# rafaelsoStanford/State_Policy_DiffusionModel

Measured on AMD Instinct MI355X. Metric: denoise-steps/sec (B=4096, horizon=32), higher is better.
Workload: dtype f32 (split-fp16 MFMA operands, fp32 accumulate)

## Files before the change

include/spdm.h:

```cpp
#ifndef SPDM_H
#define SPDM_H

#include <stddef.h>
#include <stdint.h>

#ifdef __cplusplus
extern "C" {
#endif

#define SPDM_NAME_MAX 64
#define SPDM_ABI_VERSION 2

typedef enum {
    SPDM_OK = 0,
    SPDM_ERR_INVALID = -1,
    SPDM_ERR_HIP = -2,
    SPDM_ERR_STATE = -3,
    SPDM_ERR_MISSING = -4,
    SPDM_ERR_NOMEM = -5
} spdm_status;

typedef enum { SPDM_DDPM = 0, SPDM_DDIM = 1 } spdm_scheduler_kind;

typedef struct spdm_handle spdm_handle;

typedef struct {
    int32_t horizon;
    int32_t state_dim;
    int32_t cond_dim;
    int32_t time_dim;
    int32_t attention;
    int32_t max_batch;
    int32_t device;
    int32_t num_train_timesteps;
    int32_t flags;
} spdm_config;

#define SPDM_FLAG_DEBUG_KEEP 1
#define SPDM_FLAG_EXACT_FP32 2
#define SPDM_FLAG_SIMPLE_UNET 4

#define SPDM_FLAG_TRAIN 8

#define SPDM_FLAG_TRAIN_ATTENTION 16

#define SPDM_FLAG_TRAIN_SIMPLE 32

typedef struct {
    char     name[SPDM_NAME_MAX];
    uint64_t offset;
    uint64_t numel;
    int32_t  ndim;
    int32_t  shape[4];
} spdm_tensor_index;

int  spdm_abi_version(void);
const char* spdm_last_error(void);

int  spdm_create(const spdm_config* cfg, spdm_handle** out);
void spdm_destroy(spdm_handle* h);

int  spdm_load_weights(spdm_handle* h, const float* h_blob, size_t n_floats,
                       const spdm_tensor_index* h_index, int32_t n_index);

int  spdm_update_weights(spdm_handle* h, const float* d_blob, size_t n_floats, void* stream);

int  spdm_debug_weight_digest(const spdm_handle* h, uint64_t* out);

int  spdm_set_time_table(spdm_handle* h, const float* h_table, int32_t T);

int  spdm_set_schedule(spdm_handle* h, int32_t kind, int32_t num_train_timesteps,
                       int32_t num_inference_steps, float beta_start, float beta_end);

int  spdm_set_schedule_tables(spdm_handle* h, int32_t kind, int32_t n_steps,
                              const int32_t* h_timesteps, const float* h_coef);

int  spdm_schedule_tables(int32_t kind, int32_t num_train_timesteps, int32_t num_inference_steps,
                          float beta_start, float beta_end,
                          int32_t* h_timesteps_out, float* h_coef_out );

int  spdm_unet_forward(spdm_handle* h, int32_t B, const float* d_x, const int32_t* h_t,
                       int32_t t_count, const float* d_cond, float* d_eps, void* stream);

int  spdm_sample(spdm_handle* h, int32_t B, const float* d_cond,
                 const float* d_inpaint, int32_t inp_h, int32_t inpaint_per_sample,
                 const float* d_xT, const float* d_noise, uint64_t seed, uint64_t sample_offset,
                 float* d_out, float* d_history, void* stream);

int  spdm_train_loss_grad(spdm_handle* h, int32_t B, const float* d_x_noisy, const int32_t* h_t, int32_t t_count,
                          const float* d_cond, const float* d_noise, float* d_loss, float* d_eps, float* d_grad,
                          float* d_grad_cond, void* stream);

int  spdm_train_set_time_scale(spdm_handle* h, const float* d_scale, int32_t B);

int  spdm_sample_begin(spdm_handle* h, int32_t B, const float* d_cond,
                       const float* d_inpaint, int32_t inp_h, int32_t inpaint_per_sample,
                       const float* d_xT, const float* d_noise, uint64_t seed,
                       uint64_t sample_offset, float* d_history, void* stream);
int  spdm_sample_run(spdm_handle* h, int32_t step_begin, int32_t step_end, void* stream);
int  spdm_sample_result(spdm_handle* h, float* d_out, void* stream);

int64_t spdm_graph_captures(const spdm_handle* h);

int  spdm_debug_tensor(spdm_handle* h, const char* name, float* d_out, size_t cap_floats,
                       int32_t shape_out[4]);

int32_t spdm_demoted_tensors(const spdm_handle* h);
int  spdm_nonfinite(spdm_handle* h, int32_t* flag_out, void* stream);

int  spdm_set_switch(spdm_handle* h, const char* name, int32_t on);

int32_t spdm_uses_split_precision(const spdm_handle* h);

size_t spdm_device_bytes(const spdm_handle* h);

int  spdm_profile_enable(spdm_handle* h, int32_t on);
int  spdm_profile_read(spdm_handle* h, int64_t* launches, double* total_ms, double* total_flops);

int  spdm_bench_gemm(int32_t device, int32_t B, int32_t H, int32_t W, int32_t Cin, int32_t Cout, int32_t taps,
                     int32_t pro, int32_t epi, int32_t split, int32_t iters, int32_t debug,
                     double* ms_out );

typedef struct spdm_encoder spdm_encoder;
int  spdm_encoder_create(int32_t device, const float* h_blob, size_t n_floats, const spdm_tensor_index* h_index,
                         int32_t n_index, spdm_encoder** out);
int  spdm_encoder_forward(spdm_encoder* e, int32_t n_images, const float* d_images, float* d_latent, void* stream);
void spdm_encoder_destroy(spdm_encoder* e);

int  spdm_encoder_train_forward(spdm_encoder* e, int32_t n_images, const float* d_images, float* d_latent, void* stream);
int  spdm_encoder_backward(spdm_encoder* e, int32_t n_images, const float* d_images, const float* d_grad_latent,
                           float* d_grad, void* stream);
int  spdm_encoder_update_weights(spdm_encoder* e, const float* d_blob, size_t n_floats, void* stream);

typedef struct spdm_decoder spdm_decoder;
int  spdm_decoder_create(int32_t device, const float* h_blob, size_t n_floats, const spdm_tensor_index* h_index,
                         int32_t n_index, spdm_decoder** out);
int  spdm_decoder_forward(spdm_decoder* d, int32_t n, const float* d_latent, float* d_recon, void* stream);
int  spdm_decoder_train_loss(spdm_decoder* d, int32_t n, const float* d_latent, const float* d_target,
                             float* d_recon , float* d_loss, void* stream);
int  spdm_decoder_backward(spdm_decoder* d, int32_t n, const float* d_latent, const float* d_target, float* d_grad,
                           float* d_grad_latent, void* stream);
int  spdm_decoder_update_weights(spdm_decoder* d, const float* d_blob, size_t n_floats, void* stream);
void spdm_decoder_destroy(spdm_decoder* d);

#define SPDM_OPTIM_MAX_SEGMENTS 4
typedef struct { float* d_param; const float* d_grad; float* d_exp_avg; float* d_exp_avg_sq; uint64_t numel; } spdm_optim_segment;
size_t spdm_adam_workspace_doubles(void);
int  spdm_adam_step(int32_t device, const spdm_optim_segment* h_segments, int32_t n_segments, int64_t step,
                    float lr, float beta1, float beta2, float eps, float max_norm,
                    double* d_workspace, void* stream);
size_t spdm_adam_norm_index(void);

int  spdm_debug_geometry(int32_t M, int32_t N, int32_t K, int32_t HW, int32_t W, int32_t taps, uint32_t switches,
                         int32_t out[10]);

int  spdm_op_gelu(const float* d_x, float* d_y, size_t n, void* stream);

typedef struct {
    int32_t B, H, W, K, N, taps;
    int32_t split;
    int32_t pro;
    int32_t epi;
    const float* d_src;  int32_t src_ld;
    const float* d_skip; int32_t skip_ld;  int32_t up_C;
    const float* h_weight;
    const double* d_src_stats; int32_t src_slots, src_m_tile, src_n_tiles, src_cnorm;
    const float* d_gamma; const float* d_beta;
    const double* d_skip_stats; int32_t skip_slots, skip_m_tile, skip_n_tiles, skip_cnorm;
    const float* d_skip_gamma; const float* d_skip_beta;
    const float* d_bias; const float* d_resid; int32_t resid_ld;
    float* d_dst; int32_t dst_ld;
    double* d_stats; size_t stats_cap;
    double* d_row_stats; size_t row_stats_cap;
    int32_t out[10];
} spdm_op_gemm_args;

int  spdm_op_gemm(spdm_op_gemm_args* args);

#ifdef __cplusplus
}
#endif
#endif
```

state_policy_diffusionmodel_amd/_lib.py:

```python
from __future__ import annotations

import ctypes
import os
from ctypes import POINTER, c_char_p, c_double, c_float, c_int32, c_int64, c_size_t, c_uint64, c_void_p

from .weights import TensorIndex

HERE = os.path.dirname(os.path.abspath(__file__))
LIB_PATH = os.environ.get("SPDM_LIB") or os.path.join(HERE, "libspdm_hip.so")

SPDM_DDPM, SPDM_DDIM = 0, 1
SPDM_FLAG_DEBUG_KEEP = 1
SPDM_FLAG_EXACT_FP32 = 2
SPDM_FLAG_SIMPLE_UNET = 4
SPDM_FLAG_TRAIN = 8
SPDM_FLAG_TRAIN_ATTENTION = 16
SPDM_FLAG_TRAIN_SIMPLE = 32
SPDM_ERR_INVALID = -1
SPDM_ERR_STATE = -3
ABI_VERSION = 2


class SpdmOpGemmArgs(ctypes.Structure):
    _fields_ = ([(n, c_int32) for n in ("B", "H", "W", "K", "N", "taps", "split", "pro", "epi")] +
                [("d_src", c_void_p), ("src_ld", c_int32), ("d_skip", c_void_p), ("skip_ld", c_int32), ("up_C", c_int32),
                 ("h_weight", c_void_p),
                 ("d_src_stats", c_void_p)] + [(n, c_int32) for n in ("src_slots", "src_m_tile", "src_n_tiles", "src_cnorm")] +
                [("d_gamma", c_void_p), ("d_beta", c_void_p),
                 ("d_skip_stats", c_void_p)] + [(n, c_int32) for n in ("skip_slots", "skip_m_tile", "skip_n_tiles", "skip_cnorm")] +
                [("d_skip_gamma", c_void_p), ("d_skip_beta", c_void_p),
                 ("d_bias", c_void_p), ("d_resid", c_void_p), ("resid_ld", c_int32),
                 ("d_dst", c_void_p), ("dst_ld", c_int32),
                 ("d_stats", c_void_p), ("stats_cap", c_size_t), ("d_row_stats", c_void_p), ("row_stats_cap", c_size_t),
                 ("out", c_int32 * 10)])


class SpdmOptimSegment(ctypes.Structure):
    _fields_ = [("d_param", c_void_p), ("d_grad", c_void_p), ("d_exp_avg", c_void_p), ("d_exp_avg_sq", c_void_p),
                ("numel", c_uint64)]


class SpdmConfig(ctypes.Structure):
    _fields_ = [(n, c_int32) for n in ("horizon", "state_dim", "cond_dim", "time_dim", "attention", "max_batch",
                                        "device", "num_train_timesteps", "flags")]


SYMBOLS = {
    "spdm_abi_version": (c_int32, []),
    "spdm_last_error": (c_char_p, []),
    "spdm_create": (c_int32, [POINTER(SpdmConfig), POINTER(c_void_p)]),
    "spdm_destroy": (None, [c_void_p]),
    "spdm_load_weights": (c_int32, [c_void_p, c_void_p, c_size_t, POINTER(TensorIndex), c_int32]),
    "spdm_update_weights": (c_int32, [c_void_p, c_void_p, c_size_t, c_void_p]),
    "spdm_debug_weight_digest": (c_int32, [c_void_p, POINTER(c_uint64)]),
    "spdm_set_time_table": (c_int32, [c_void_p, c_void_p, c_int32]),
    "spdm_set_schedule": (c_int32, [c_void_p, c_int32, c_int32, c_int32, c_float, c_float]),
    "spdm_set_schedule_tables": (c_int32, [c_void_p, c_int32, c_int32, c_void_p, c_void_p]),
    "spdm_schedule_tables": (c_int32, [c_int32, c_int32, c_int32, c_float, c_float, c_void_p, c_void_p]),
    "spdm_unet_forward": (c_int32, [c_void_p, c_int32, c_void_p, c_void_p, c_int32, c_void_p, c_void_p, c_void_p]),
    "spdm_sample": (c_int32, [c_void_p, c_int32, c_void_p, c_void_p, c_int32, c_int32, c_void_p, c_void_p, c_uint64,
                              c_uint64, c_void_p, c_void_p, c_void_p]),
    "spdm_train_loss_grad": (c_int32, [c_void_p, c_int32, c_void_p, c_void_p, c_int32, c_void_p, c_void_p, c_void_p, c_void_p,
                                       c_void_p, c_void_p, c_void_p]),
    "spdm_train_set_time_scale": (c_int32, [c_void_p, c_void_p, c_int32]),
    "spdm_sample_begin": (c_int32, [c_void_p, c_int32, c_void_p, c_void_p, c_int32, c_int32, c_void_p, c_void_p,
                                    c_uint64, c_uint64, c_void_p, c_void_p]),
    "spdm_sample_run": (c_int32, [c_void_p, c_int32, c_int32, c_void_p]),
    "spdm_sample_result": (c_int32, [c_void_p, c_void_p, c_void_p]),
    "spdm_graph_captures": (c_int64, [c_void_p]),
    "spdm_debug_tensor": (c_int32, [c_void_p, c_char_p, c_void_p, c_size_t, POINTER(c_int32 * 4)]),
    "spdm_uses_split_precision": (c_int32, [c_void_p]),
    "spdm_demoted_tensors": (c_int32, [c_void_p]),
    "spdm_nonfinite": (c_int32, [c_void_p, POINTER(c_int32), c_void_p]),
    "spdm_set_switch": (c_int32, [c_void_p, c_char_p, c_int32]),
    "spdm_device_bytes": (c_size_t, [c_void_p]),
    "spdm_profile_enable": (c_int32, [c_void_p, c_int32]),
    "spdm_profile_read": (c_int32, [c_void_p, POINTER(c_int64), POINTER(c_double), POINTER(c_double)]),
    "spdm_encoder_create": (c_int32, [c_int32, c_void_p, c_size_t, POINTER(TensorIndex), c_int32, POINTER(c_void_p)]),
    "spdm_encoder_forward": (c_int32, [c_void_p, c_int32, c_void_p, c_void_p, c_void_p]),
    "spdm_encoder_destroy": (None, [c_void_p]),
    "spdm_encoder_train_forward": (c_int32, [c_void_p, c_int32, c_void_p, c_void_p, c_void_p]),
    "spdm_encoder_backward": (c_int32, [c_void_p, c_int32, c_void_p, c_void_p, c_void_p, c_void_p]),
    "spdm_encoder_update_weights": (c_int32, [c_void_p, c_void_p, c_size_t, c_void_p]),
    "spdm_decoder_create": (c_int32, [c_int32, c_void_p, c_size_t, POINTER(TensorIndex), c_int32, POINTER(c_void_p)]),
    "spdm_decoder_forward": (c_int32, [c_void_p, c_int32, c_void_p, c_void_p, c_void_p]),
    "spdm_decoder_train_loss": (c_int32, [c_void_p, c_int32, c_void_p, c_void_p, c_void_p, c_void_p, c_void_p]),
    "spdm_decoder_backward": (c_int32, [c_void_p, c_int32, c_void_p, c_void_p, c_void_p, c_void_p, c_void_p]),
    "spdm_decoder_update_weights": (c_int32, [c_void_p, c_void_p, c_size_t, c_void_p]),
    "spdm_decoder_destroy": (None, [c_void_p]),
    "spdm_adam_workspace_doubles": (c_size_t, []),
    "spdm_adam_step": (c_int32, [c_int32, POINTER(SpdmOptimSegment), c_int32, c_int64, c_float, c_float, c_float, c_float, c_float,
                                 c_void_p, c_void_p]),
    "spdm_adam_norm_index": (c_size_t, []),
    "spdm_op_gelu": (c_int32, [c_void_p, c_void_p, c_size_t, c_void_p]),
    "spdm_op_gemm": (c_int32, [POINTER(SpdmOpGemmArgs)]),
    "spdm_debug_geometry": (c_int32, [c_int32] * 6 + [ctypes.c_uint32, POINTER(c_int32 * 10)]),
    "spdm_bench_gemm": (c_int32, [c_int32] * 12 + [POINTER(c_double)]),
}

_lib = None


def load() -> ctypes.CDLL:
    global _lib
    if _lib is not None:
        return _lib
    if not os.path.exists(LIB_PATH):
        raise RuntimeError(
            f"{LIB_PATH} not found: the HIP extension has not been built "
            "(run `python -m state_policy_diffusionmodel_amd.build`); there is no CPU fallback")
    import torch
    lib = ctypes.CDLL(LIB_PATH)
    for name, (res, args) in SYMBOLS.items():
        try:
            fn = getattr(lib, name)
        except AttributeError as e:
            raise RuntimeError(f"{LIB_PATH} does not export {name}") from e
        fn.restype = res
        fn.argtypes = args
    if lib.spdm_abi_version() != ABI_VERSION:
        raise RuntimeError(f"ABI version mismatch: library {lib.spdm_abi_version()}, binding {ABI_VERSION}")
    _lib = lib
    return lib


def check(rc: int, what: str) -> None:
    if rc != 0:
        msg = load().spdm_last_error()
        raise RuntimeError(f"{what} failed ({rc}): {msg.decode() if msg else '?'}")
```

state_policy_diffusionmodel_amd/csrc/conv_wide.hip:

```cpp
#include <algorithm>
#include <cstdlib>

#include "device_utils.h"

namespace spdm {

typedef float f32x16 __attribute__((ext_vector_type(16)));
typedef float f32x4 __attribute__((ext_vector_type(4)));
typedef float f32x2 __attribute__((ext_vector_type(2)));
typedef _Float16 f16x8 __attribute__((ext_vector_type(8)));
typedef _Float16 f16x2 __attribute__((ext_vector_type(2)));

namespace {

constexpr float ACT_SCALE = 16.0f;
constexpr float DESCALE = 1.0f / 2048.0f;
constexpr int CK = 32;
#ifndef WIDE_LDS_PERM
#define WIDE_LDS_PERM 1
#endif
template <bool W2, bool PIPE = false, bool WP = false> struct WidePitch { static constexpr int value = (W2 || PIPE || WP || !WIDE_LDS_PERM) ? 36 : 40; };
constexpr bool wp_active(int t, int rt) { return !((t % 3 == 0 && (rt & 3) == 0) || (t % 3 == 2 && (rt & 3) == 3)); }
constexpr int wp_first(int t) { return (t % 3 == 0) ? 1 : 0; }
constexpr int wp_next(int t, int rt, int RT) {
    for (int r = rt + 1; r < RT; ++r)
        if (wp_active(t, r)) return r;
    return -1;
}
constexpr int wp_order(int t, int rt, int RT) {
    int n = 0;
    for (int tt = 0; tt < t; ++tt)
        for (int r = 0; r < RT; ++r) n += wp_active(tt, r) ? 1 : 0;
    for (int r = 0; r < rt; ++r) n += wp_active(t, r) ? 1 : 0;
    return n;
}
#ifndef WIDE_STAGE_GROUP
#define WIDE_STAGE_GROUP 1
#endif
#ifndef WIDE_DB
#define WIDE_DB 0
#endif
#ifndef WIDE_EARLY
#define WIDE_EARLY 0
#endif
#ifndef WIDE_NH
#define WIDE_NH 2
#endif

__device__ __forceinline__ f32x2 split2(float a, float b) {
    unsigned h, l;
    split_pair_f16(a * ACT_SCALE, b * ACT_SCALE, h, l);
    return f32x2{__builtin_bit_cast(float, h), __builtin_bit_cast(float, l)};
}

template <int NT, int PRO, bool W2, int RT, int WN, bool PIPE, bool TWO = false, int WP = 0, bool G2 = false>
#ifndef WIDE_MINB
#define WIDE_MINB 2
#endif
__global__ __launch_bounds__(256, WIDE_MINB) void conv3x3_wide_kernel(const GemmArgs a, const int epi_slots, const int NS) {
    constexpr int WM = 4 / WN;
    constexpr int CT = 2 * NT;
    constexpr int RW = RT * 16;
    constexpr int NTHR = 256;
    constexpr int RP = NTHR / 8;
    constexpr int M_T = WM * RW, N_T = WN * NT * 32;
    constexpr int APASS = (M_T + 18 + RP - 1) / RP;
    constexpr int FAR = (W2 || WP) ? 4 : 3;
    constexpr int FBR = (NT == 2) ? 2 : 3;
    constexpr int PH = 3 * NT;
    constexpr int BB = (APASS <= 9) ? 7 : (APASS <= 10) ? 6 : 5;
    static_assert(APASS * BB <= 64, "sample-index packing");
    static_assert(!W2 || NT == 2, "the width-2 variant exists for 128-wide tiles");
    static_assert(RT == 8 || (RT == 4 && NT == 2 && !W2), "64-row waves only in the tap-pair loop");
    static_assert(WN == 2 || (WN == 1 && RT == 4), "the 4 x 1 wave arrangement uses 64-row waves");
    static_assert(!TWO || (!PIPE && PRO != PRO_GN_GELU), "two-source input: first conv of a block, plain hand-over");
    static_assert(WP == 0 || WP == 4 || WP == 8, "row permutation for width-4 or width-8 maps");
    static_assert(!WP || (NT == 2 && WN == 2 && !W2 && !PIPE), "row permutation: 128-wide tiles");
    static_assert((16 + 4 * (WP == 8 ? 7 : 6)) % 4 == 0, "A ring phase");
    static_assert(WP != 8 || RT == 8, "width-8 maps: one 128-row block per wave");
    constexpr bool WP8 = (WP == 8);
    constexpr int NI8 = (M_T + 18 + 6) / 8 + 1;
    static_assert(!G2 || (NT == 2 && RT == 4 && !W2 && !PIPE && !WP && !WIDE_DB), "two chunks per hand-over: the plain tap loop, 64 rows per wave");
    extern __shared__ __attribute__((aligned(16))) float smem[];

    const int tid = threadIdx.x, lane = tid & 63;
    const int wave = __builtin_amdgcn_readfirstlane(tid >> 6);
    const int wm = wave / WN, wn = wave % WN, l16 = lane & 15, kg = lane >> 4;
    const int HW = a.HW, W = a.W, H = a.H, M = a.M, K = a.K, N = a.N;
    const int halo = W + 1;
    const int QA = M_T + 2 * halo;
    const int QZ = WP8 ? 8 * NI8 + 2 : QA + 2;

    const int n_ntiles = N / N_T;
    const int nblk = gridDim.x, bid = blockIdx.x;
    const int q8 = nblk >> 3, r8 = nblk & 7, xcd = bid & 7, idx = bid >> 3;
    const int logical = (xcd < r8 ? xcd * (q8 + 1) : r8 * (q8 + 1) + (xcd - r8) * q8) + idx;
    const int ksp = a.ksplit > 1 ? a.ksplit : 1;
    const int tiles_mn = nblk / ksp;
    const int ks = logical / tiles_mn, tl = logical - ks * tiles_mn;
    const int mtile = tl / n_ntiles, ntile = tl - mtile * n_ntiles;
    const int m0 = mtile * M_T, n0 = ntile * N_T;
    const int kc0 = 2 * (int)((long long)ks * (K / (2 * CK)) / ksp), kc1 = (ksp > 1) ? 2 * (int)((long long)(ks + 1) * (K / (2 * CK)) / ksp) : K / CK;

    static_assert(!PIPE || (NT == 2 && !W2), "the pipelined hand-over exists in the tap loop of 128-wide tiles");
    constexpr int LDK = WidePitch<W2, PIPE, (WP != 0) || G2>::value;
    constexpr bool PERM = WIDE_LDS_PERM && !W2 && !PIPE && !WP && !G2;
    constexpr bool DB = PIPE || (WIDE_DB && (NT == 2) && !W2);
    float* Abuf = smem;
    float* Awr = smem + (DB ? QZ * LDK : 0);
    float* smean = smem + ((DB || G2) ? 2 : 1) * QZ * LDK;
    float* srstd = smean + NS;

#ifdef SPDM_DIAG
    const bool stamping = (a.debug & DBG_STAMP) && a.stamps != nullptr && tid == 0;
#define WIDE_STAMP(k_) if (stamping) a.stamps[(size_t)bid * 8 + (k_)] = (unsigned long long)__builtin_amdgcn_s_memtime();
    if (stamping) {
        a.stamps[(size_t)bid * 8 + 0] = (unsigned long long)__builtin_amdgcn_s_memrealtime();
        a.stamps[(size_t)bid * 8 + 6] = (unsigned long long)__builtin_amdgcn_s_getreg(63492);
        a.stamps[(size_t)bid * 8 + 7] = (unsigned long long)__builtin_amdgcn_s_getreg(63508);
    }
    const bool dbg_no_mfma = (a.debug & DBG_NO_MFMA) != 0, dbg_no_wload = (a.debug & DBG_NO_WLOAD) != 0;
    const bool dbg_no_aload = (a.debug & DBG_NO_ALOAD) != 0;
#else
#define WIDE_STAMP(k_)
    constexpr bool dbg_no_mfma = false, dbg_no_wload = false, dbg_no_aload = false;
#endif
    WIDE_STAMP(1)
    const int zrow = WP8 ? 8 * NI8 : QA;
    if (tid < LDK) { Abuf[zrow * LDK + tid] = 0.f; Awr[zrow * LDK + tid] = 0.f; }
    if (G2 && tid < LDK) Abuf[(QZ + QA) * LDK + tid] = 0.f;

    constexpr bool pro = (PRO != PRO_NONE);
    constexpr bool pro_gelu = (PRO == PRO_GN_GELU);
    int bh_first = 0;
    if (pro) {
        const int lo = max(m0 - halo, 0), hi = min(m0 + M_T + halo, M) - 1;
        bh_first = lo / HW;
        const int bh_last = hi / HW;
        for (int t = tid; t <= bh_last - bh_first; t += NTHR) {
            float mean, rstd;
            sample_mean_rstd(a.pro_stats, bh_first + t, mean, rstd);
            smean[t] = mean;
            srstd[t] = rstd;
        }
        __syncthreads();
    }

    const int srow_t = tid >> 3, c4 = tid & 7;
    unsigned avalid = 0u;
    unsigned long long abidx = 0ull;
#pragma unroll
    for (int p = 0; p < APASS; ++p) {
        const int q = p * RP + srow_t;
        const int m = m0 - halo + q;
        const bool v = (q < QA) && (m >= 0) && (m < M);
        if (v) {
            avalid |= 1u << p;
            if (pro) abidx |= (unsigned long long)(m / HW - bh_first) << (BB * p);
        }
    }
    const float* abase = a.src + c4 * 4;
    const float* abase1 = TWO ? a.skip + c4 * 4 : nullptr;
    const int nc0 = TWO ? a.up_C / CK : 0;
    bool ident = false;

#define WIDE_ROWOFF(rt_) (W2 ? (((rt_) >> 1) * 32 + ((rt_) & 1)) : WP8 ? (rt_) : WP ? (((rt_) >> 2) * 64 + ((rt_) & 3)) : (rt_) * 16)
#define WIDE_LDSOFF(rt_) (WP8 ? (rt_) * NI8 : WIDE_ROWOFF(rt_))
    const int rowlane = W2 ? 2 * l16 : WP ? WP * l16 : PERM ? (l16 < 4 ? l16 : l16 < 12 ? l16 + 4 : l16 - 8) : l16;
    const int aoff0 = WP8 ? (2 + wm * 16 + l16) * LDK + kg * 4 : (wm * RW + rowlane + halo) * LDK + kg * 4;
    const int zoff = zrow * LDK + kg * 4;
    unsigned am[(RT + 2) / 3] = {};
#pragma unroll
    for (int rt = 0; rt < RT; ++rt) {
        const int m = m0 + wm * RW + WIDE_ROWOFF(rt) + rowlane;
        unsigned mask = 0u;
        if (m < M) {
            const int p = m % HW;
            const int h = p / W, w = p - h * W;
#pragma unroll
            for (int t = 0; t < 9; ++t) {
                const int dh = t / 3 - 1, dw = t % 3 - 1;
                const bool ok = (h + dh >= 0) && (h + dh < H) && (w + dw >= 0) && (w + dw < W);
                mask |= (ok ? 1u : 0u) << t;
            }
        }
        am[rt / 3] |= mask << (9 * (rt % 3));
    }
    const int nchunks = K / CK;
    const float* wfl = a.wgt_frag + ((size_t)((n0 >> 4) + wn * CT) * 2) * 256 + lane * 4;
    const size_t wtap = (size_t)(N >> 4) * 2 * 256;

    f32x4 acc[RT][CT];
#pragma unroll
    for (int rt = 0; rt < RT; ++rt)
#pragma unroll
        for (int ct = 0; ct < CT; ++ct) acc[rt][ct] = f32x4{0.f, 0.f, 0.f, 0.f};

    f32x4 areg[APASS];
    f32x4 g4r = {1.f, 1.f, 1.f, 1.f}, b4r = {0.f, 0.f, 0.f, 0.f};

    int srow_o = srow_t;
#ifdef WIDE_NO_OPAQUE
#define WIDE_OPAQUE_ROW
#else
#define WIDE_OPAQUE_ROW if constexpr (PRO != PRO_NONE && RT == 8) asm volatile("" : "+v"(srow_o));
#endif
#define WIDE_LOAD_A(chunk_) WIDE_LOAD_A_(chunk_, areg, g4r, b4r, ident)
#define WIDE_STAGE_A() WIDE_STAGE_A_(areg, g4r, b4r, ident, Awr)
#define WIDE_LOAD_A_(chunk_, areg_, g4r_, b4r_, ident_)                                              \
    {                                                                                                \
        WIDE_OPAQUE_ROW                                                                              \
        const bool first_ = !TWO || (chunk_) < nc0;                                                  \
        const int cc_ = (TWO && !first_) ? (chunk_) - nc0 : (chunk_);       \
        const float* ab_ = (first_ ? abase : abase1) + cc_ * CK;                                     \
        const int ld_ = first_ ? a.src_ld : a.skip_ld;                                               \
        _Pragma("unroll") for (int p_ = 0; p_ < APASS; ++p_) {                                      \
            const int mc_ = min(max(m0 - halo + p_ * RP + srow_o, 0), M - 1);                        \
            areg_[p_] = *reinterpret_cast<const f32x4*>(ab_ + (size_t)mc_ * ld_);                     \
        }                                                                                            \
        if (pro) {                                                                                   \
            ident_ = TWO && first_;                                                                   \
            g4r_ = *reinterpret_cast<const f32x4*>(a.pro_gamma + cc_ * CK + c4 * 4);                  \
            b4r_ = *reinterpret_cast<const f32x4*>(a.pro_beta + cc_ * CK + c4 * 4);                   \
            if (TWO && first_) { g4r_ = f32x4{1.f, 1.f, 1.f, 1.f}; b4r_ = f32x4{0.f, 0.f, 0.f, 0.f}; } \
        }                                                                                            \
    }
#define WIDE_STAGE_A_(areg_, g4r_, b4r_, ident_, dst_)                                                                             \
    {                                                                                                \
        _Pragma("unroll") for (int p_ = 0; p_ < APASS; ++p_) {                                      \
            f32x4 v_ = areg_[p_];                                                                     \
            if (pro) {                                                                               \
                const int bi_ = (int)((abidx >> (BB * p_)) & ((1ull << BB) - 1));                                  \
                float rs_ = srstd[bi_], mu_ = smean[bi_];                                            \
                if (TWO && ident_) { rs_ = 1.f; mu_ = 0.f; }        \
                v_.x = (v_.x - mu_) * (rs_ * g4r_.x) + b4r_.x;                                         \
                v_.y = (v_.y - mu_) * (rs_ * g4r_.y) + b4r_.y;                                         \
                v_.z = (v_.z - mu_) * (rs_ * g4r_.z) + b4r_.z;                                         \
                v_.w = (v_.w - mu_) * (rs_ * g4r_.w) + b4r_.w;                                         \
                if (pro_gelu) {                                                                      \
                    v_.x = gelu_erf(v_.x); v_.y = gelu_erf(v_.y);                                    \
                    v_.z = gelu_erf(v_.z); v_.w = gelu_erf(v_.w);                                    \
                }                                                                                    \
            }                                                                                        \
            if (!((avalid >> p_) & 1u)) v_ = f32x4{0.f, 0.f, 0.f, 0.f};                              \
            const f32x2 p0_ = split2(v_.x, v_.y), p1_ = split2(v_.z, v_.w);                          \
            {                    \
                const int q_ = p_ * RP + srow_o;                                                     \
                float* row_ = (dst_) + (WP8 ? (q_ < QA ? ((q_ + 7) & 7) * NI8 + ((q_ + 7) >> 3) : 8 * NI8 + 1) : min(q_, QA + 1)) * LDK; \
                *reinterpret_cast<f32x2*>(row_ + c4 * 2) = f32x2{p0_.x, p1_.x};              \
                *reinterpret_cast<f32x2*>(row_ + 16 + c4 * 2) = f32x2{p0_.y, p1_.y};         \
            }                                                                                        \
            if (pro && (p_ % WIDE_STAGE_GROUP) == WIDE_STAGE_GROUP - 1) __builtin_amdgcn_sched_barrier(0);    \
        }                                                                                            \
    }
#define WIDE_LOAD_B(slot_, chunk_, tap_, cp_)                                                        \
    if (!dbg_no_wload) {                                                                             \
        const float* p_ = wfl + (size_t)((tap_) * nchunks + (chunk_)) * wtap + (cp_) * 1024;         \
        _Pragma("unroll") for (int c_ = 0; c_ < 2; ++c_) {                                          \
            fb[slot_][c_][0] = *reinterpret_cast<const f16x8*>(p_ + c_ * 512);                       \
            fb[slot_][c_][1] = *reinterpret_cast<const f16x8*>(p_ + c_ * 512 + 256);                 \
        }                                                                                            \
    }
#define WIDE_LOAD_FA(slot_, tap_, shift_, rt_)                                                       \
    {                                                                                                \
        const unsigned mb_ = (am[(rt_) / 3] >> (9 * ((rt_) % 3) + (tap_))) & 1u;                     \
        const int o_ = mb_ ? aoff0 + WIDE_LDSOFF(rt_) * LDK + (shift_) : zoff;                       \
        fa[slot_][0] = *reinterpret_cast<const f16x8*>(Abuf + o_);                                   \
        fa[slot_][1] = *reinterpret_cast<const f16x8*>(Abuf + o_ + 16);                              \
    }
#define WIDE_STEP(fas_, fbs_, rt_, ct0_)                                                             \
    if (!dbg_no_mfma) {                                                                              \
        acc[rt_][(ct0_)] = __builtin_amdgcn_mfma_f32_16x16x32_f16(fa[fas_][0], fb[fbs_][0][0], acc[rt_][(ct0_)], 0, 0, 0);         \
        acc[rt_][(ct0_) + 1] = __builtin_amdgcn_mfma_f32_16x16x32_f16(fa[fas_][0], fb[fbs_][1][0], acc[rt_][(ct0_) + 1], 0, 0, 0); \
        acc[rt_][(ct0_)] = __builtin_amdgcn_mfma_f32_16x16x32_f16(fa[fas_][0], fb[fbs_][0][1], acc[rt_][(ct0_)], 0, 0, 0);         \
        acc[rt_][(ct0_) + 1] = __builtin_amdgcn_mfma_f32_16x16x32_f16(fa[fas_][0], fb[fbs_][1][1], acc[rt_][(ct0_) + 1], 0, 0, 0); \
        acc[rt_][(ct0_)] = __builtin_amdgcn_mfma_f32_16x16x32_f16(fa[fas_][1], fb[fbs_][0][0], acc[rt_][(ct0_)], 0, 0, 0);         \
        acc[rt_][(ct0_) + 1] = __builtin_amdgcn_mfma_f32_16x16x32_f16(fa[fas_][1], fb[fbs_][1][0], acc[rt_][(ct0_) + 1], 0, 0, 0); \
    }

    const int nrows = (kc1 - kc0) * 3;
    f16x8 fa[FAR][2], fb[FBR][2][2];
#define WIDE_SHIFT(kr_, dwi_) (WP8 ? (((dwi_) - 1) * NI8 + ((kr_) - 1)) * LDK : (((kr_) - 1) * W + ((dwi_) - 1)) * LDK)

    if constexpr (!W2 && NT == 2 && !(WP && RT == 8)) {
        f16x8 fbt[2][4][2], fat[2][2];
#define TAP_LOAD_B(slot_, chunk_, tap_)                                                              \
        if (!dbg_no_wload) {                                                                         \
            const float* p_ = wfl + (size_t)((tap_) * nchunks + (chunk_)) * wtap;                    \
            _Pragma("unroll") for (int c_ = 0; c_ < 4; ++c_) {                                      \
                fbt[slot_][c_][0] = *reinterpret_cast<const f16x8*>(p_ + c_ * 512);                  \
                fbt[slot_][c_][1] = *reinterpret_cast<const f16x8*>(p_ + c_ * 512 + 256);            \
            }                                                                                        \
        }
#define TAP_LOAD_FA(slot_, tap_, shift_, rt_)                                                        \
        {                                                                                            \
            const unsigned mb_ = (am[(rt_) / 3] >> (9 * ((rt_) % 3) + (tap_))) & 1u;                 \
            const int o_ = mb_ ? aoff0 + WIDE_ROWOFF(rt_) * LDK + (shift_) : zoff;                   \
            fat[slot_][0] = *reinterpret_cast<const f16x8*>(Abuf + o_);                              \
            fat[slot_][1] = *reinterpret_cast<const f16x8*>(Abuf + o_ + 16);                         \
        }
        const int TAPS = a.taps;
        const bool t3 = (TAPS == 3);
#define TAP_SHIFT(tap_) (t3 ? ((tap_) - 1) * W * LDK : (((tap_) / 3 - 1) * W + ((tap_) - ((tap_) / 3) * 3 - 1)) * LDK)
#define TAP_BIT(tap_) (t3 ? 3 * (tap_) + 1 : (tap_))
        if constexpr (WP) {
#define WP_SHIFT(t_) ((((t_) / 3 - 1) * W + ((t_) % 3 - 1)) * LDK)
            TAP_LOAD_B(0, kc0, 0)
            WIDE_LOAD_A(kc0)
            WIDE_STAGE_A()
            __syncthreads();
            WIDE_STAMP(2)
            int aoff_w = aoff0;
#define WP_LOAD_FA(slot_, tap_, shift_, rt_)                                                         \
            {                                                                                        \
                const unsigned mb_ = (am[(rt_) / 3] >> (9 * ((rt_) % 3) + (tap_))) & 1u;             \
                const int o_ = mb_ ? aoff_w + WIDE_ROWOFF(rt_) * LDK + (shift_) : zoff;              \
                fat[slot_][0] = *reinterpret_cast<const f16x8*>(Abuf + o_);                          \
                fat[slot_][1] = *reinterpret_cast<const f16x8*>(Abuf + o_ + 16);                     \
            }
            WP_LOAD_FA(0, 0, WP_SHIFT(0), wp_first(0))
            for (int chunk = kc0; chunk < kc1; ++chunk) {
                const int cn1 = min(chunk + 1, kc1 - 1);
                asm volatile("" : "+v"(aoff_w));
#pragma unroll
                for (int i = 0; i < (RT + 2) / 3; ++i) asm volatile("" : "+v"(am[i]));
#pragma unroll
                for (int t = 0; t < 9; ++t) {
                    if (t < 8) { TAP_LOAD_B((t + 1) & 1, chunk, t + 1) } else { TAP_LOAD_B(1, cn1, 0) }
#pragma unroll
                    for (int rt = 0; rt < RT; ++rt) {
                        {
                            if (wp_active(t, rt)) {
                                const int g = wp_order(t, rt, RT);
                                const int nx = wp_next(t, rt, RT);
                                if (nx >= 0) { WP_LOAD_FA((g + 1) & 1, t, WP_SHIFT(t), nx) }
                                else if (t < 8) { WP_LOAD_FA((g + 1) & 1, t + 1, WP_SHIFT(t + 1), wp_first(t + 1)) }
                                __builtin_amdgcn_sched_barrier(0);
                                if (!dbg_no_mfma) {
#pragma unroll
                                    for (int c = 0; c < 4; ++c)
                                        acc[rt][c] = __builtin_amdgcn_mfma_f32_16x16x32_f16(fat[g & 1][0], fbt[t & 1][c][0], acc[rt][c], 0, 0, 0);
#pragma unroll
                                    for (int c = 0; c < 4; ++c)
                                        acc[rt][c] = __builtin_amdgcn_mfma_f32_16x16x32_f16(fat[g & 1][0], fbt[t & 1][c][1], acc[rt][c], 0, 0, 0);
#pragma unroll
                                    for (int c = 0; c < 4; ++c)
                                        acc[rt][c] = __builtin_amdgcn_mfma_f32_16x16x32_f16(fat[g & 1][1], fbt[t & 1][c][0], acc[rt][c], 0, 0, 0);
                                }
                                __builtin_amdgcn_sched_barrier(0);
                            }
                        }
                    }
                }
                if (chunk + 1 < kc1 && !dbg_no_aload) {
                    WIDE_LOAD_A(chunk + 1)
                    __syncthreads();
                    WIDE_STAGE_A()
                    __syncthreads();
                }
#pragma unroll
                for (int c = 0; c < 4; ++c) { fbt[0][c][0] = fbt[1][c][0]; fbt[0][c][1] = fbt[1][c][1]; }
                WP_LOAD_FA(0, 0, WP_SHIFT(0), wp_first(0))
            }
#undef WP_SHIFT
#undef WP_LOAD_FA
        } else if constexpr (PIPE) {
            f32x4 ar[3];
            int pm0 = m0 - halo + srow_t, srow_p = srow_t, aoff_p = aoff0;
#define PIPE_OPAQUE() asm volatile("" : "+v"(pm0), "+v"(srow_p), "+v"(aoff_p));
#define PIPE_LOAD_FA(slot_, tap_, shift_, rt_)                                                       \
            {                                                                                        \
                const unsigned mb_ = (am[(rt_) / 3] >> (9 * ((rt_) % 3) + (tap_))) & 1u;             \
                const int o_ = mb_ ? aoff_p + WIDE_ROWOFF(rt_) * LDK + (shift_) : zoff;              \
                fat[slot_][0] = *reinterpret_cast<const f16x8*>(Abuf + o_);                          \
                fat[slot_][1] = *reinterpret_cast<const f16x8*>(Abuf + o_ + 16);                     \
            }
#define PIPE_LOAD(slot_, chunk_, pass_)                                                              \
            {                                                                                        \
                const int mc_ = min(max(pm0 + (pass_) * RP, 0), M - 1);                              \
                ar[slot_] = *reinterpret_cast<const f32x4*>(abase + (size_t)mc_ * a.src_ld + (chunk_) * CK); \
            }
#define PIPE_GB(chunk_)                                                                              \
            if (pro) {                                                                               \
                g4r = *reinterpret_cast<const f32x4*>(a.pro_gamma + (chunk_) * CK + c4 * 4);         \
                b4r = *reinterpret_cast<const f32x4*>(a.pro_beta + (chunk_) * CK + c4 * 4);          \
            }
#define PIPE_STAGE(slot_, pass_)                                                                     \
            {                                                                                        \
                f32x4 v_ = ar[slot_];                                                                \
                if (pro) {                                                                           \
                    const int bi_ = (int)((abidx >> (BB * (pass_))) & ((1ull << BB) - 1));           \
                    const float rs_ = srstd[bi_], mu_ = smean[bi_];                                  \
                    v_.x = (v_.x - mu_) * (rs_ * g4r.x) + b4r.x;                                     \
                    v_.y = (v_.y - mu_) * (rs_ * g4r.y) + b4r.y;                                     \
                    v_.z = (v_.z - mu_) * (rs_ * g4r.z) + b4r.z;                                     \
                    v_.w = (v_.w - mu_) * (rs_ * g4r.w) + b4r.w;                                     \
                    if (pro_gelu) {                                                                  \
                        v_.x = gelu_erf(v_.x); v_.y = gelu_erf(v_.y);                                \
                        v_.z = gelu_erf(v_.z); v_.w = gelu_erf(v_.w);                                \
                    }                                                                                \
                }                                                                                    \
                if (!((avalid >> (pass_)) & 1u)) v_ = f32x4{0.f, 0.f, 0.f, 0.f};                     \
                const f32x2 p0_ = split2(v_.x, v_.y), p1_ = split2(v_.z, v_.w);                      \
                float* row_ = Awr + min((pass_) * RP + srow_p, QA + 1) * LDK;                        \
                *reinterpret_cast<f32x2*>(row_ + c4 * 2) = f32x2{p0_.x, p1_.x};                      \
                *reinterpret_cast<f32x2*>(row_ + 16 + c4 * 2) = f32x2{p0_.y, p1_.y};                 \
            }
#define PIPE_SHIFT(t_) ((((t_) / 3 - 1) * W + ((t_) % 3 - 1)) * LDK)
            TAP_LOAD_B(0, kc0, 0)
            WIDE_LOAD_A(kc0)
            WIDE_STAGE_A()
            __syncthreads();
            { float* t_ = Abuf; Abuf = Awr; Awr = t_; }
            {
                const int c1 = min(kc0 + 1, kc1 - 1);
                PIPE_LOAD(0, c1, 0)
                PIPE_LOAD(1, c1, 1)
                PIPE_LOAD(2, c1, 2)
                PIPE_GB(c1)
            }
            WIDE_STAMP(2)
            PIPE_LOAD_FA(0, 0, PIPE_SHIFT(0), 0)
            for (int chunk = kc0; chunk < kc1; ++chunk) {
                const int cn1 = min(chunk + 1, kc1 - 1), cn2 = min(chunk + 2, kc1 - 1);
                PIPE_OPAQUE()
#pragma unroll
                for (int t = 0; t < 9; ++t) {
                    if (t < 8) { TAP_LOAD_B((t + 1) & 1, chunk, t + 1) } else { TAP_LOAD_B(1, cn1, 0) }
                    if (t < APASS) { PIPE_STAGE(t % 3, t) }
                    if (t + 3 < APASS) { PIPE_LOAD(t % 3, cn1, t + 3) }
                    else if (t >= 6) { PIPE_LOAD(t - 6, cn2, t - 6) }
                    if (t == 8) { PIPE_GB(cn2) }
#pragma unroll
                    for (int rt = 0; rt < RT; ++rt) {
                        if (rt + 1 < RT) { PIPE_LOAD_FA((rt + 1) & 1, t, PIPE_SHIFT(t), rt + 1) }
                        else if (t < 8) { PIPE_LOAD_FA(0, t + 1, PIPE_SHIFT(t + 1), 0) }
                        __builtin_amdgcn_sched_barrier(0);
#pragma unroll
                        for (int c = 0; c < 4; ++c)
                            acc[rt][c] = __builtin_amdgcn_mfma_f32_16x16x32_f16(fat[rt & 1][0], fbt[t & 1][c][0], acc[rt][c], 0, 0, 0);
#pragma unroll
                        for (int c = 0; c < 4; ++c)
                            acc[rt][c] = __builtin_amdgcn_mfma_f32_16x16x32_f16(fat[rt & 1][0], fbt[t & 1][c][1], acc[rt][c], 0, 0, 0);
#pragma unroll
                        for (int c = 0; c < 4; ++c)
                            acc[rt][c] = __builtin_amdgcn_mfma_f32_16x16x32_f16(fat[rt & 1][1], fbt[t & 1][c][0], acc[rt][c], 0, 0, 0);
                        __builtin_amdgcn_sched_barrier(0);
                    }
                }
                __syncthreads();
                { float* t_ = Abuf; Abuf = Awr; Awr = t_; }
#pragma unroll
                for (int c = 0; c < 4; ++c) { fbt[0][c][0] = fbt[1][c][0]; fbt[0][c][1] = fbt[1][c][1]; }
                PIPE_LOAD_FA(0, 0, PIPE_SHIFT(0), 0)
            }
#undef PIPE_OPAQUE
#undef PIPE_LOAD_FA
#undef PIPE_LOAD
#undef PIPE_GB
#undef PIPE_STAGE
#undef PIPE_SHIFT
        } else if constexpr (G2) {
        const int ntaps = (kc1 - kc0) * TAPS;
        f32x4 areg2[APASS];
        f32x4 g4r2 = {1.f, 1.f, 1.f, 1.f}, b4r2 = {0.f, 0.f, 0.f, 0.f};
        bool ident2 = false;
        const float* Acur = Abuf;
#define G2_LOAD_FA(slot_, tap_, shift_, rt_)                                                         \
        {                                                                                            \
            const unsigned mb_ = (am[(rt_) / 3] >> (9 * ((rt_) % 3) + (tap_))) & 1u;                 \
            const int o_ = mb_ ? aoff0 + WIDE_ROWOFF(rt_) * LDK + (shift_) : zoff;                   \
            fat[slot_][0] = *reinterpret_cast<const f16x8*>(Acur + o_);                              \
            fat[slot_][1] = *reinterpret_cast<const f16x8*>(Acur + o_ + 16);                         \
        }
        TAP_LOAD_B(0, kc0, 0)
        WIDE_LOAD_A_(kc0, areg, g4r, b4r, ident)
        WIDE_LOAD_A_(min(kc0 + 1, kc1 - 1), areg2, g4r2, b4r2, ident2)
        WIDE_STAGE_A_(areg, g4r, b4r, ident, Abuf)
        WIDE_STAGE_A_(areg2, g4r2, b4r2, ident2, Abuf + QZ * LDK)
        __syncthreads();
        WIDE_STAMP(2)
        G2_LOAD_FA(0, TAP_BIT(0), TAP_SHIFT(0), 0)
        int chunk = kc0, tap = 0;
        for (int tt = 0; tt < ntaps; tt += 2) {
#pragma unroll
            for (int half = 0; half < 2; ++half) {
                int ntap = tap + 1, nchunk = chunk;
                if (ntap == TAPS) { ntap = 0; nchunk = chunk + 1; }
                const bool have_next = (tt + half + 1 < ntaps);
                const bool next_C = have_next && (ntap == 0);
                const bool next_A = next_C && (((nchunk - kc0) & 1) == 0);
                TAP_LOAD_B(1 - half, (have_next ? nchunk : chunk), (have_next ? ntap : tap))
                const int sh = TAP_SHIFT(tap), nsh = TAP_SHIFT(ntap), tb = TAP_BIT(tap), ntb = TAP_BIT(ntap);
#pragma unroll
                for (int rt = 0; rt < RT; ++rt) {
                    if (rt + 1 < RT) { G2_LOAD_FA((rt + 1) & 1, tb, sh, rt + 1) }
                    else if (have_next && !next_C) { G2_LOAD_FA(0, ntb, nsh, 0) }
                    __builtin_amdgcn_sched_barrier(0);
                    if (!dbg_no_mfma) {
#pragma unroll
                        for (int c = 0; c < 4; ++c)
                            acc[rt][c] = __builtin_amdgcn_mfma_f32_16x16x32_f16(fat[rt & 1][0], fbt[half][c][0], acc[rt][c], 0, 0, 0);
#pragma unroll
                        for (int c = 0; c < 4; ++c)
                            acc[rt][c] = __builtin_amdgcn_mfma_f32_16x16x32_f16(fat[rt & 1][0], fbt[half][c][1], acc[rt][c], 0, 0, 0);
#pragma unroll
                        for (int c = 0; c < 4; ++c)
                            acc[rt][c] = __builtin_amdgcn_mfma_f32_16x16x32_f16(fat[rt & 1][1], fbt[half][c][0], acc[rt][c], 0, 0, 0);
                    }
                    __builtin_amdgcn_sched_barrier(0);
                }
                if (next_A && !dbg_no_aload) {
                    WIDE_LOAD_A_(nchunk, areg, g4r, b4r, ident)
                    WIDE_LOAD_A_(min(nchunk + 1, kc1 - 1), areg2, g4r2, b4r2, ident2)
                    __syncthreads();
                    WIDE_STAGE_A_(areg, g4r, b4r, ident, Abuf)
                    WIDE_STAGE_A_(areg2, g4r2, b4r2, ident2, Abuf + QZ * LDK)
                    __syncthreads();
                    Acur = Abuf;
                    G2_LOAD_FA(0, TAP_BIT(0), TAP_SHIFT(0), 0)
                } else if (next_C) {
                    Acur = Abuf + (dbg_no_aload ? 0 : ((nchunk - kc0) & 1) * QZ * LDK);
                    G2_LOAD_FA(0, TAP_BIT(0), TAP_SHIFT(0), 0)
                }
                tap = ntap;
                chunk = nchunk;
            }
        }
#undef G2_LOAD_FA
        } else {
        const int ntaps = (kc1 - kc0) * TAPS;
        TAP_LOAD_B(0, kc0, 0)
        WIDE_LOAD_A(kc0)
        WIDE_STAGE_A()
        __syncthreads();
        if (DB) { float* t_ = Abuf; Abuf = Awr; Awr = t_; }
        WIDE_STAMP(2)
        TAP_LOAD_FA(0, TAP_BIT(0), TAP_SHIFT(0), 0)
        int chunk = kc0, tap = 0;
        for (int tt = 0; tt < ntaps; tt += 2) {
#pragma unroll
            for (int half = 0; half < 2; ++half) {
                int ntap = tap + 1, nchunk = chunk;
                if (ntap == TAPS) { ntap = 0; nchunk = chunk + 1; }
                const bool have_next = (tt + half + 1 < ntaps);
                const bool next_A = have_next && (ntap == 0);
                TAP_LOAD_B(1 - half, (have_next ? nchunk : chunk), (have_next ? ntap : tap))
                const int sh = TAP_SHIFT(tap), nsh = TAP_SHIFT(ntap), tb = TAP_BIT(tap), ntb = TAP_BIT(ntap);
                if (DB && WIDE_EARLY && next_A && !dbg_no_aload) { WIDE_LOAD_A(nchunk) }
#pragma unroll
                for (int rt = 0; rt < RT; ++rt) {
                    if (rt + 1 < RT) { TAP_LOAD_FA((rt + 1) & 1, tb, sh, rt + 1) }
                    else if (have_next && !next_A) { TAP_LOAD_FA(0, ntb, nsh, 0) }
                    __builtin_amdgcn_sched_barrier(0);
                    if (!dbg_no_mfma) {
#pragma unroll
                        for (int c = 0; c < 4; ++c)
                            acc[rt][c] = __builtin_amdgcn_mfma_f32_16x16x32_f16(fat[rt & 1][0], fbt[half][c][0], acc[rt][c], 0, 0, 0);
#pragma unroll
                        for (int c = 0; c < 4; ++c)
                            acc[rt][c] = __builtin_amdgcn_mfma_f32_16x16x32_f16(fat[rt & 1][0], fbt[half][c][1], acc[rt][c], 0, 0, 0);
#pragma unroll
                        for (int c = 0; c < 4; ++c)
                            acc[rt][c] = __builtin_amdgcn_mfma_f32_16x16x32_f16(fat[rt & 1][1], fbt[half][c][0], acc[rt][c], 0, 0, 0);
                    }
                    __builtin_amdgcn_sched_barrier(0);
                }
                if (next_A && !dbg_no_aload) {
                    if (!(DB && WIDE_EARLY)) { WIDE_LOAD_A(nchunk) }
                    if (!DB) __syncthreads();
                    WIDE_STAGE_A()
                    __syncthreads();
                    if (DB) { float* t_ = Abuf; Abuf = Awr; Awr = t_; }
                    TAP_LOAD_FA(0, TAP_BIT(0), TAP_SHIFT(0), 0)
                } else if (next_A) {
                    TAP_LOAD_FA(0, TAP_BIT(0), TAP_SHIFT(0), 0)
                }
                tap = ntap;
                chunk = nchunk;
            }
        }
        }
#undef TAP_LOAD_B
#undef TAP_LOAD_FA
#undef TAP_SHIFT
#undef TAP_BIT
    } else if constexpr (WP) {
#define WP_PLUS(i_) (WP8 ? (i_) : (i_) + (i_) / 3)
#define WP_MINUS(i_) (WP8 ? (i_) + 1 : (i_) + (i_) / 3 + 1)
        constexpr int WS = WP8 ? 7 : 6;
        constexpr int Q1 = 16 + 2 * WS, Q2 = 16 + 4 * WS;
        WIDE_LOAD_B(0, kc0, 1, 0)
        WIDE_LOAD_A(kc0)
        WIDE_STAGE_A()
        __syncthreads();
        WIDE_STAMP(2)
        WIDE_LOAD_FA(0, 1, WIDE_SHIFT(0, 1), 0)
        WIDE_LOAD_FA(1, 1, WIDE_SHIFT(0, 1), 1)
        int chunk = kc0, kr = 0;
        for (int r = 0; r < nrows; ++r) {
            int nkr = kr + 1, nchunk = chunk;
            if (nkr == 3) { nkr = 0; nchunk = chunk + 1; }
            const bool have_next = (r + 1 < nrows);
            const bool next_A = have_next && (nkr == 0);
            const int bkr = have_next ? nkr : kr, bchunk = have_next ? nchunk : chunk;
#pragma unroll
            for (int cp = 0; cp < 2; ++cp) {
                if (cp == 0) { WIDE_LOAD_B(1, chunk, kr * 3 + 1, 1) } else { WIDE_LOAD_B(0, chunk, kr * 3 + 2, 0) }
#pragma unroll
                for (int rt = 0; rt < RT; ++rt) {
                    const int q = cp * 8 + rt;
                    if (q + 2 < 16) { WIDE_LOAD_FA((q + 2) % FAR, kr * 3 + 1, WIDE_SHIFT(kr, 1), (q + 2) % 8) }
                    else { WIDE_LOAD_FA((q + 2) % FAR, kr * 3 + 2, WIDE_SHIFT(kr, 2), WP_PLUS(q + 2 - 16)) }
                    __builtin_amdgcn_sched_barrier(0);
                    WIDE_STEP(q % FAR, cp, rt, cp * 2)
                    __builtin_amdgcn_sched_barrier(0);
                }
            }
#pragma unroll
            for (int cp = 0; cp < 2; ++cp) {
                if (cp == 0) { WIDE_LOAD_B(1, chunk, kr * 3 + 2, 1) } else { WIDE_LOAD_B(0, chunk, kr * 3, 0) }
#pragma unroll
                for (int i = 0; i < WS; ++i) {
                    const int q = 16 + cp * WS + i;
                    if (q + 2 < Q1) { WIDE_LOAD_FA((q + 2) % FAR, kr * 3 + 2, WIDE_SHIFT(kr, 2), WP_PLUS((q + 2 - 16) % WS)) }
                    else { WIDE_LOAD_FA((q + 2) % FAR, kr * 3, WIDE_SHIFT(kr, 0), WP_MINUS(q + 2 - Q1)) }
                    __builtin_amdgcn_sched_barrier(0);
                    WIDE_STEP(q % FAR, cp, WP_PLUS(i), cp * 2)
                    __builtin_amdgcn_sched_barrier(0);
                }
            }
#pragma unroll
            for (int cp = 0; cp < 2; ++cp) {
                if (cp == 0) { WIDE_LOAD_B(1, chunk, kr * 3, 1) } else { WIDE_LOAD_B(0, bchunk, bkr * 3 + 1, 0) }
#pragma unroll
                for (int i = 0; i < WS; ++i) {
                    const int q = Q1 + cp * WS + i;
                    if (q + 2 < Q2) { WIDE_LOAD_FA((q + 2) % FAR, kr * 3, WIDE_SHIFT(kr, 0), WP_MINUS((q + 2 - Q1) % WS)) }
                    else if (have_next && !next_A) { WIDE_LOAD_FA((q + 2) % FAR, nkr * 3 + 1, WIDE_SHIFT(nkr, 1), q + 2 - Q2) }
                    __builtin_amdgcn_sched_barrier(0);
                    WIDE_STEP(q % FAR, cp, WP_MINUS(i), cp * 2)
                    __builtin_amdgcn_sched_barrier(0);
                }
            }
            if (next_A) {
                WIDE_LOAD_A(nchunk)
                __syncthreads();
                WIDE_STAGE_A()
                __syncthreads();
                WIDE_LOAD_FA(0, 1, WIDE_SHIFT(0, 1), 0)
                WIDE_LOAD_FA(1, 1, WIDE_SHIFT(0, 1), 1)
            }
            kr = nkr;
            chunk = nchunk;
        }
#undef WP_PLUS
#undef WP_MINUS
    } else if constexpr (!W2) {
        WIDE_LOAD_B(0, kc0, 0, 0)
        WIDE_LOAD_A(kc0)
        WIDE_STAGE_A()
        __syncthreads();
        WIDE_STAMP(2)
        WIDE_LOAD_FA(0, 0, WIDE_SHIFT(0, 0), 0)
        WIDE_LOAD_FA(1, 0, WIDE_SHIFT(0, 0), 1)
        int chunk = kc0, kr = 0;
        for (int r = 0; r < nrows; ++r) {
            int nkr = kr + 1, nchunk = chunk;
            if (nkr == 3) { nkr = 0; nchunk = chunk + 1; }
            const bool have_next = (r + 1 < nrows);
            const bool next_A = have_next && (nkr == 0);
            const int bkr = have_next ? nkr : kr, bchunk = have_next ? nchunk : chunk;
#pragma unroll
            for (int ph = 0; ph < PH; ++ph) {
                if (ph + 1 < PH) {
                    WIDE_LOAD_B((ph + 1) % FBR, chunk, kr * 3 + (ph + 1) / NT, (ph + 1) % NT)
                } else {
                    WIDE_LOAD_B((ph + 1) % FBR, bchunk, bkr * 3, 0)
                }
#pragma unroll
                for (int rt = 0; rt < RT; ++rt) {
                    const int G = ph * RT + rt;
                    if (G + 2 < PH * RT) {
                        const int dwi2 = ((G + 2) / RT) / NT;
                        WIDE_LOAD_FA((G + 2) % FAR, kr * 3 + dwi2, WIDE_SHIFT(kr, dwi2), (G + 2) % RT)
                    } else if (have_next && !next_A) {
                        WIDE_LOAD_FA((G + 2) % FAR, nkr * 3, WIDE_SHIFT(nkr, 0), G + 2 - PH * RT)
                    }
                    __builtin_amdgcn_sched_barrier(0);
                    WIDE_STEP(G % FAR, ph % FBR, rt, (ph % NT) * 2)
                    __builtin_amdgcn_sched_barrier(0);
                }
            }
            if (next_A) {
                WIDE_LOAD_A(nchunk)
                __syncthreads();
                WIDE_STAGE_A()
                __syncthreads();
                WIDE_LOAD_FA(0, 0, WIDE_SHIFT(0, 0), 0)
                WIDE_LOAD_FA(1, 0, WIDE_SHIFT(0, 0), 1)
            }
            kr = nkr;
            chunk = nchunk;
        }
    } else {
        WIDE_LOAD_B(0, kc0, 1, 0)
        WIDE_LOAD_A(kc0)
        WIDE_STAGE_A()
        __syncthreads();
        WIDE_STAMP(2)
        WIDE_LOAD_FA(0, 1, WIDE_SHIFT(0, 1), 0)
        WIDE_LOAD_FA(1, 1, WIDE_SHIFT(0, 1), 1)
        int chunk = kc0, kr = 0;
        for (int r = 0; r < nrows; ++r) {
            int nkr = kr + 1, nchunk = chunk;
            if (nkr == 3) { nkr = 0; nchunk = chunk + 1; }
            const bool have_next = (r + 1 < nrows);
            const bool next_A = have_next && (nkr == 0);
            const int bkr = have_next ? nkr : kr, bchunk = have_next ? nchunk : chunk;
#pragma unroll
            for (int cp = 0; cp < 2; ++cp) {
                if (cp == 0) { WIDE_LOAD_B(1, chunk, kr * 3 + 1, 1) } else { WIDE_LOAD_B(0, chunk, kr * 3 + 2, 0) }
#pragma unroll
                for (int rt = 0; rt < RT; ++rt) {
                    const int q = cp * 8 + rt;
                    if (q + 2 < 16) { WIDE_LOAD_FA((q + 2) % FAR, kr * 3 + 1, WIDE_SHIFT(kr, 1), (q + 2) % 8) }
                    else { WIDE_LOAD_FA((q + 2) % FAR, kr * 3 + 2, WIDE_SHIFT(kr, 2), 2 * (q + 2 - 16)) }
                    __builtin_amdgcn_sched_barrier(0);
                    WIDE_STEP(q % FAR, cp, rt, cp * 2)
                    __builtin_amdgcn_sched_barrier(0);
                }
            }
#pragma unroll
            for (int cp = 0; cp < 2; ++cp) {
                if (cp == 0) { WIDE_LOAD_B(1, chunk, kr * 3 + 2, 1) } else { WIDE_LOAD_B(0, chunk, kr * 3, 0) }
#pragma unroll
                for (int i = 0; i < 4; ++i) {
                    const int q = 16 + cp * 4 + i;
                    if (q + 2 < 24) { WIDE_LOAD_FA((q + 2) % FAR, kr * 3 + 2, WIDE_SHIFT(kr, 2), 2 * ((q + 2 - 16) % 4)) }
                    else { WIDE_LOAD_FA((q + 2) % FAR, kr * 3, WIDE_SHIFT(kr, 0), 2 * (q + 2 - 24) + 1) }
                    __builtin_amdgcn_sched_barrier(0);
                    WIDE_STEP(q % FAR, cp, 2 * i, cp * 2)
                    __builtin_amdgcn_sched_barrier(0);
                }
            }
#pragma unroll
            for (int cp = 0; cp < 2; ++cp) {
                if (cp == 0) { WIDE_LOAD_B(1, chunk, kr * 3, 1) } else { WIDE_LOAD_B(0, bchunk, bkr * 3 + 1, 0) }
#pragma unroll
                for (int i = 0; i < 4; ++i) {
                    const int q = 24 + cp * 4 + i;
                    if (q + 2 < 32) { WIDE_LOAD_FA((q + 2) % FAR, kr * 3, WIDE_SHIFT(kr, 0), 2 * ((q + 2 - 24) % 4) + 1) }
                    else if (have_next && !next_A) { WIDE_LOAD_FA((q + 2) % FAR, nkr * 3 + 1, WIDE_SHIFT(nkr, 1), q + 2 - 32) }
                    __builtin_amdgcn_sched_barrier(0);
                    WIDE_STEP(q % FAR, cp, 2 * i + 1, cp * 2)
                    __builtin_amdgcn_sched_barrier(0);
                }
            }
            if (next_A) {
                WIDE_LOAD_A(nchunk)
                __syncthreads();
                WIDE_STAGE_A()
                __syncthreads();
                WIDE_LOAD_FA(0, 1, WIDE_SHIFT(0, 1), 0)
                WIDE_LOAD_FA(1, 1, WIDE_SHIFT(0, 1), 1)
            }
            kr = nkr;
            chunk = nchunk;
        }
    }
#undef WIDE_LOAD_A
#undef WIDE_STAGE_A
#undef WIDE_LOAD_B
#undef WIDE_LOAD_FA
#undef WIDE_STEP
#undef WIDE_SHIFT
    WIDE_STAMP(3)
    __syncthreads();

#pragma unroll
    for (int rt = 0; rt < RT; ++rt)
#pragma unroll
        for (int ct = 0; ct < CT; ++ct) acc[rt][ct] *= DESCALE;

    const int rb4 = PERM ? ((0x1320 >> (4 * kg)) & 0xF) : kg;
    constexpr int NH = W2 ? 2 : WP ? RT / 4 : WIDE_NH;
    constexpr int HROWS = M_T / NH;
    const bool partial_out = ksp > 1;
    float* const dstp = partial_out ? a.partial + (size_t)ks * M * N : a.dst;
    const int dst_ld = partial_out ? N : a.dst_ld;
    float* otile = smem;
    float* srow = smem + HROWS * N_T;
#pragma unroll
    for (int rt = 0; rt < RT; ++rt) {
        const int unit = wm * (RW / 4) + (W2 ? (rt >> 1) * 8 + 2 * kg + (rt & 1) : WP8 ? 8 * kg + rt : WP ? (rt >> 2) * 16 + 4 * kg + (rt & 3) : rt * 4 + rb4);
        float s1 = 0.f, s2 = 0.f;
#pragma unroll
        for (int ct = 0; ct < CT; ++ct)
#pragma unroll
            for (int j = 0; j < 4; ++j) {
                const float v = acc[rt][ct][j];
                s1 += v;
                s2 += v * v;
            }
        s1 = row16_sum_dpp(s1);
        s2 = row16_sum_dpp(s2);
        if (l16 == 0) {
            srow[(unit * WN + wn) * 2] = s1;
            srow[(unit * WN + wn) * 2 + 1] = s2;
        }
    }

#pragma unroll
    for (int h = 0; h < NH; ++h) {
        if (h) __syncthreads();
        if constexpr (WP8) {
#pragma unroll
            for (int rt = 0; rt < RT; ++rt)
#pragma unroll
                for (int ct = 0; ct < CT; ++ct) {
                    const int col_l = wn * NT * 32 + ct * 16 + l16;
                    if ((kg >> 1) == h) {
#pragma unroll
                        for (int j = 0; j < 4; ++j)
                            otile[(wm * (RW / NH) + 8 * (4 * (kg & 1) + j) + rt) * N_T + col_l] = acc[rt][ct][j];
                    }
                }
        } else
#pragma unroll
        for (int rq = 0; rq < RT / NH; ++rq) {
            const int rt = (RT / NH) * h + rq;
#pragma unroll
            for (int ct = 0; ct < CT; ++ct) {
                const int col_l = wn * NT * 32 + ct * 16 + l16;
#pragma unroll
                for (int j = 0; j < 4; ++j) {
                    const int rw = W2 ? ((rt >> 1) - 2 * h) * 32 + 2 * (4 * kg + j) + (rt & 1) : WP ? 4 * (4 * kg + j) + (rt & 3) : rq * 16 + 4 * rb4 + j;
                    otile[(wm * (RW / NH) + rw) * N_T + col_l] = acc[rt][ct][j];
                }
            }
        }
        __syncthreads();
        if (h == 0) WIDE_STAMP(4)
        if (h == 0 && !partial_out) {
            const int t_lo = m0, t_hi = min(m0 + M_T, M);
            const int ups = HW >> 2;
            const bool whole = (HW % M_T == 0);
            const bool aligned = whole || (M_T % HW == 0 && (ups & (ups - 1)) == 0);
            if (aligned) {
                if (wave == 0) {
                    constexpr int NU = M_T / 4;
                    const int u = lane, uc = min(lane, NU - 1);
                    double d1 = 0.0, d2 = 0.0;
#pragma unroll
                    for (int w2 = 0; w2 < WN; ++w2) {
                        d1 += (double)srow[(uc * WN + w2) * 2];
                        d2 += (double)srow[(uc * WN + w2) * 2 + 1];
                    }
                    const int seg = whole ? NU : ups;
                    d1 = seg_sum_f64(d1, seg);
                    d2 = seg_sum_f64(d2, seg);
                    const int row = t_lo + 4 * u;
                    if (u < NU && (u & (seg - 1)) == 0 && row < t_hi) {
                        const int b = row / HW;
                        const int slot = (mtile - (b * HW) / M_T) * n_ntiles + ntile;
                        double* o = a.epi_stats + ((size_t)b * epi_slots + slot) * 2;
                        o[0] = d1;
                        o[1] = d2;
                    }
                }
            } else if (t_hi > t_lo) {
                const int b_first = t_lo / HW, b_last = (t_hi - 1) / HW;
                for (int t = tid; t <= b_last - b_first; t += NTHR) {
                    const int b = b_first + t;
                    const int r_lo = max(b * HW, t_lo) - m0, r_hi = min((b + 1) * HW, t_hi) - m0;
                    double s1 = 0.0, s2 = 0.0;
                    for (int u = r_lo >> 2; u < ((r_hi + 3) >> 2); ++u)
                        for (int w2 = 0; w2 < WN; ++w2) {
                            s1 += (double)srow[(u * WN + w2) * 2];
                            s2 += (double)srow[(u * WN + w2) * 2 + 1];
                        }
                    const int slot = (mtile - (b * HW) / M_T) * n_ntiles + ntile;
                    double* o = a.epi_stats + ((size_t)b * epi_slots + slot) * 2;
                    o[0] = s1;
                    o[1] = s2;
                }
            }
        }
        constexpr int TPR = N_T / 4, RPP = NTHR / TPR;
        const int c4o = tid % TPR, r0 = tid / TPR;
#pragma unroll 4
        for (int p = 0; p < HROWS / RPP; ++p) {
            const int lr = p * RPP + r0;
            const int row = m0 + (lr / (RW / NH)) * RW + h * (RW / NH) + lr % (RW / NH);
            if (row < M) {
                const f32x4 v = *reinterpret_cast<const f32x4*>(otile + lr * N_T + c4o * 4);
                *reinterpret_cast<f32x4*>(dstp + (size_t)row * dst_ld + n0 + c4o * 4) = v;
            }
        }
    }
    WIDE_STAMP(5)
#undef WIDE_STAMP
#undef WIDE_ROWOFF
}

template <int NT, int PRO, bool W2 = false, int RT = 8, int WN = 2, bool PIPE = false, bool TWO = false, int WP = 0, bool G2 = false>
hipError_t launch_wide_cfg(const GemmArgs& a, const GemmGeom& g, hipStream_t s) {
    constexpr int M_T = (4 / WN) * RT * 16, N_T = WN * 32 * NT, NTHR = 256;
    constexpr int APASS = (M_T + 18 + 31) / 32, NSMAX = (APASS <= 9) ? 128 : (APASS <= 10) ? 64 : 32;
    const int halo = a.W + 1;
    const int QA = M_T + 2 * halo;
    const int NS = (((QA - 1) / a.HW + 2) + 3) & ~3;
    if (NS > NSMAX || g.m_tile != M_T || g.n_tile != N_T) return hipErrorInvalidValue;
    constexpr bool DB = PIPE || (WIDE_DB && (NT == 2) && !W2);
    constexpr int LDK = WidePitch<W2, PIPE, (WP != 0) || G2>::value;
    if (PIPE && a.taps != 9) return hipErrorInvalidValue;
    if (WP && (a.taps != 9 || a.W != WP || a.HW % (4 * WP) != 0)) return hipErrorInvalidValue;
    const int QZ = (WP == 8) ? 8 * ((M_T + 18 + 6) / 8 + 1) + 2 : QA + 2;
    size_t lds = (size_t)(((DB || G2) ? 2 : 1) * QZ * LDK + 2 * NS) * sizeof(float);
    lds = std::max(lds, (size_t)((M_T / (W2 ? 2 : WP ? RT / 4 : WIDE_NH)) * N_T + (M_T / 4) * WN * 2) * sizeof(float));
    if (lds > 160 * 1024) return hipErrorInvalidValue;
    auto kern = conv3x3_wide_kernel<NT, PRO, W2, RT, WN, PIPE, TWO, WP, G2>;
    if (hipError_t e = allow_full_lds(reinterpret_cast<const void*>(kern)); e != hipSuccess) return e;
    const int n_mtiles = (a.M + M_T - 1) / M_T;
    if (a.ksplit > 1 && a.K % 64 != 0) return hipErrorInvalidValue;
    if (a.route) *a.route = GemmRoute{ROUTE_WIDE, WP == 4 ? VAR_WP4 : WP == 8 ? VAR_WP8 : W2 ? VAR_W2 : PIPE ? VAR_PIPE : G2 ? VAR_G2 : VAR_PLAIN, M_T, N_T};
    hipLaunchKernelGGL(kern, dim3(n_mtiles * g.n_tiles * std::max(a.ksplit, 1)), dim3(NTHR), lds, s, a, g.slots, NS);
    return hipGetLastError();
}

}

static bool wide_w2(const GemmArgs& a) { return a.W == 2 && a.taps == 9 && !(a.sw & SW_NO_W2); }

bool conv_wide_supported(const GemmArgs& a, const GemmGeom& g) {
    const bool common = a.split && a.wgt_frag != nullptr && a.W >= 1 && a.W <= 8 && (a.HW & 3) == 0 && a.M % a.HW == 0 &&
                        a.epi == EPI_STATS && a.row_stats == nullptr && a.K % CK == 0 &&
                        (a.debug & ~(DBG_STAMP | DBG_NO_MFMA | DBG_NO_WLOAD | DBG_NO_ALOAD)) == 0 && !(a.sw & SW_NO_WIDE);
    if (!common || a.pro > PRO_GN_GELU) return false;
    if (a.skip != nullptr) {
        if (a.pro == PRO_GN_GELU || a.up_C <= 0 || a.up_C >= a.K || a.up_C % CK != 0 || g.n_tile != 128 || a.skip_ld % 4 != 0 ||
            a.skip_ld < a.K - a.up_C || a.src_ld < a.up_C) return false;
    }
    if (a.ksplit > 1 && a.K % 64 != 0) return false;
    if ((g.m_tile + 2 * (a.W + 1) - 1) / a.HW + 2 > 128) return false;
    if (g.m_tile == 128)
        return g.n_tile == 128 && (a.taps == 9 || (a.taps == 3 && a.W == 1)) && a.K % 64 == 0 && !(a.sw & SW_NO_WIDE128);
    if (g.m_tile != 256) return false;
    if (a.taps == 3) return false;
    if (a.taps != 9 || !(g.n_tile == 128 || g.n_tile == 64)) return false;
    if (wide_w2(a)) return g.n_tile == 128 && (a.HW & 7) == 0;
    if (g.n_tile == 128 && a.K % 64 != 0) return false;
    return true;
}

hipError_t launch_conv_wide(const GemmArgs& a, const GemmGeom& g, hipStream_t s) {
    if (!conv_wide_supported(a, g)) return hipErrorInvalidValue;
    const bool pipe = a.taps == 9 && a.K >= 256 && !(a.sw & SW_NO_WIDE_PIPE);
    if (a.W == 4 && a.taps == 9 && g.n_tile == 128 && a.HW % 16 == 0 && a.K % 64 == 0 && !(a.sw & SW_NO_WP4)) {
        const bool two = a.skip != nullptr;
        if (g.m_tile == 128) {
            if (two) {
                if (a.pro == PRO_NONE) return launch_wide_cfg<2, PRO_NONE, false, 4, 2, false, true, 4>(a, g, s);
                return launch_wide_cfg<2, PRO_GN, false, 4, 2, false, true, 4>(a, g, s);
            }
            if (a.pro == PRO_NONE) return launch_wide_cfg<2, PRO_NONE, false, 4, 2, false, false, 4>(a, g, s);
            if (a.pro == PRO_GN) return launch_wide_cfg<2, PRO_GN, false, 4, 2, false, false, 4>(a, g, s);
            return launch_wide_cfg<2, PRO_GN_GELU, false, 4, 2, false, false, 4>(a, g, s);
        }
        if (two) {
            if (a.pro == PRO_NONE) return launch_wide_cfg<2, PRO_NONE, false, 8, 2, false, true, 4>(a, g, s);
            return launch_wide_cfg<2, PRO_GN, false, 8, 2, false, true, 4>(a, g, s);
        }
        if (a.pro == PRO_NONE) return launch_wide_cfg<2, PRO_NONE, false, 8, 2, false, false, 4>(a, g, s);
        if (a.pro == PRO_GN) return launch_wide_cfg<2, PRO_GN, false, 8, 2, false, false, 4>(a, g, s);
        return launch_wide_cfg<2, PRO_GN_GELU, false, 8, 2, false, false, 4>(a, g, s);
    }
    if (a.W == 8 && a.taps == 9 && g.n_tile == 128 && g.m_tile == 256 && a.HW % 32 == 0 && a.K % 64 == 0 && !(a.sw & SW_NO_WP8)) {
        if (a.skip != nullptr) {
            if (a.pro == PRO_NONE) return launch_wide_cfg<2, PRO_NONE, false, 8, 2, false, true, 8>(a, g, s);
            return launch_wide_cfg<2, PRO_GN, false, 8, 2, false, true, 8>(a, g, s);
        }
        if (a.pro == PRO_NONE) return launch_wide_cfg<2, PRO_NONE, false, 8, 2, false, false, 8>(a, g, s);
        if (a.pro == PRO_GN) return launch_wide_cfg<2, PRO_GN, false, 8, 2, false, false, 8>(a, g, s);
        return launch_wide_cfg<2, PRO_GN_GELU, false, 8, 2, false, false, 8>(a, g, s);
    }
    if (a.skip != nullptr) {
        if (g.m_tile == 128) {
            if (a.pro == PRO_NONE) return launch_wide_cfg<2, PRO_NONE, false, 4, 2, false, true>(a, g, s);
            return launch_wide_cfg<2, PRO_GN, false, 4, 2, false, true>(a, g, s);
        }
        if (wide_w2(a)) {
            if (a.pro == PRO_NONE) return launch_wide_cfg<2, PRO_NONE, true, 8, 2, false, true>(a, g, s);
            return launch_wide_cfg<2, PRO_GN, true, 8, 2, false, true>(a, g, s);
        }
        if (a.pro == PRO_NONE) return launch_wide_cfg<2, PRO_NONE, false, 8, 2, false, true>(a, g, s);
        return launch_wide_cfg<2, PRO_GN, false, 8, 2, false, true>(a, g, s);
    }
    const bool g2 = a.K >= 64 && (a.sw & SW_G2);
    if (g.m_tile == 128) {
        if (g2) {
            if (a.pro == PRO_NONE) return launch_wide_cfg<2, PRO_NONE, false, 4, 2, false, false, false, true>(a, g, s);
            if (a.pro == PRO_GN) return launch_wide_cfg<2, PRO_GN, false, 4, 2, false, false, false, true>(a, g, s);
            return launch_wide_cfg<2, PRO_GN_GELU, false, 4, 2, false, false, false, true>(a, g, s);
        }
        if (a.pro == PRO_NONE) return launch_wide_cfg<2, PRO_NONE, false, 4>(a, g, s);
        if (a.pro == PRO_GN) return launch_wide_cfg<2, PRO_GN, false, 4>(a, g, s);
        return launch_wide_cfg<2, PRO_GN_GELU, false, 4>(a, g, s);
    }
    if (wide_w2(a)) {
        if (a.pro == PRO_NONE) return launch_wide_cfg<2, PRO_NONE, true>(a, g, s);
        if (a.pro == PRO_GN) return launch_wide_cfg<2, PRO_GN, true>(a, g, s);
        return launch_wide_cfg<2, PRO_GN_GELU, true>(a, g, s);
    }
    if (g.n_tile == 128) {
        if (a.pro == PRO_NONE) return launch_wide_cfg<2, PRO_NONE>(a, g, s);
        if (a.pro == PRO_GN) return launch_wide_cfg<2, PRO_GN>(a, g, s);
        return launch_wide_cfg<2, PRO_GN_GELU>(a, g, s);
    }
    if (a.K % 64 == 0 && !(a.sw & SW_WIDE_N64_2X2)) {
        if (pipe) {
            if (a.pro == PRO_NONE) return launch_wide_cfg<2, PRO_NONE, false, 4, 1, true>(a, g, s);
            if (a.pro == PRO_GN) return launch_wide_cfg<2, PRO_GN, false, 4, 1, true>(a, g, s);
            return launch_wide_cfg<2, PRO_GN_GELU, false, 4, 1, true>(a, g, s);
        }
        if (g2) {
            if (a.pro == PRO_NONE) return launch_wide_cfg<2, PRO_NONE, false, 4, 1, false, false, false, true>(a, g, s);
            if (a.pro == PRO_GN) return launch_wide_cfg<2, PRO_GN, false, 4, 1, false, false, false, true>(a, g, s);
            return launch_wide_cfg<2, PRO_GN_GELU, false, 4, 1, false, false, false, true>(a, g, s);
        }
        if (a.pro == PRO_NONE) return launch_wide_cfg<2, PRO_NONE, false, 4, 1>(a, g, s);
        if (a.pro == PRO_GN) return launch_wide_cfg<2, PRO_GN, false, 4, 1>(a, g, s);
        return launch_wide_cfg<2, PRO_GN_GELU, false, 4, 1>(a, g, s);
    }
    if (a.pro == PRO_NONE) return launch_wide_cfg<1, PRO_NONE>(a, g, s);
    if (a.pro == PRO_GN) return launch_wide_cfg<1, PRO_GN>(a, g, s);
    return launch_wide_cfg<1, PRO_GN_GELU>(a, g, s);
}

}
```

state_policy_diffusionmodel_amd/csrc/device_utils.h:

```cpp
#pragma once
#include <hip/hip_runtime.h>
#include "kernels.h"

namespace spdm {

__device__ __forceinline__ void sample_mean_rstd(const StatsRef& st, int b, float& mean, float& rstd) {
    const long long r0 = (long long)b * st.HW;
    const int first = (int)(r0 / st.m_tile);
    const int last = (int)((r0 + st.HW - 1) / st.m_tile);
    const int n = (last - first + 1) * st.n_tiles;
    const double* p = st.p + (size_t)b * st.slots * 2;
    double s1 = 0.0, s2 = 0.0;
    for (int i = 0; i < n; ++i) { s1 += p[2 * i]; s2 += p[2 * i + 1]; }
    const double m = s1 * st.inv_count;
    double var = s2 * st.inv_count - m * m;
    if (var < 0.0) var = 0.0;
    mean = (float)m;
    rstd = (float)(1.0 / sqrt(var + 1e-5));
}

__device__ __forceinline__ float sum_xor32(float v) {
    const unsigned u = __builtin_bit_cast(unsigned, v);
    const auto r = __builtin_amdgcn_permlane32_swap(u, u, false, false);
    return __builtin_bit_cast(float, (unsigned)r[0]) + __builtin_bit_cast(float, (unsigned)r[1]);
}
__device__ __forceinline__ float max_xor32(float v) {
    const unsigned u = __builtin_bit_cast(unsigned, v);
    const auto r = __builtin_amdgcn_permlane32_swap(u, u, false, false);
    return fmaxf(__builtin_bit_cast(float, (unsigned)r[0]), __builtin_bit_cast(float, (unsigned)r[1]));
}
__device__ __forceinline__ float sum_xor16(float v) {
    const unsigned u = __builtin_bit_cast(unsigned, v);
    const auto r = __builtin_amdgcn_permlane16_swap(u, u, false, false);
    return __builtin_bit_cast(float, (unsigned)r[0]) + __builtin_bit_cast(float, (unsigned)r[1]);
}
__device__ __forceinline__ double sum_xor32_f64(double v) {
    const unsigned long long u = __builtin_bit_cast(unsigned long long, v);
    const unsigned lo = (unsigned)u, hi = (unsigned)(u >> 32);
    const auto rl = __builtin_amdgcn_permlane32_swap(lo, lo, false, false);
    const auto rh = __builtin_amdgcn_permlane32_swap(hi, hi, false, false);
    const double a = __builtin_bit_cast(double, ((unsigned long long)(unsigned)rh[0] << 32) | (unsigned)rl[0]);
    const double b = __builtin_bit_cast(double, ((unsigned long long)(unsigned)rh[1] << 32) | (unsigned)rl[1]);
    return a + b;
}
__device__ __forceinline__ double sum_xor16_f64(double v) {
    const unsigned long long u = __builtin_bit_cast(unsigned long long, v);
    const unsigned lo = (unsigned)u, hi = (unsigned)(u >> 32);
    const auto rl = __builtin_amdgcn_permlane16_swap(lo, lo, false, false);
    const auto rh = __builtin_amdgcn_permlane16_swap(hi, hi, false, false);
    const double a = __builtin_bit_cast(double, ((unsigned long long)(unsigned)rh[0] << 32) | (unsigned)rl[0]);
    const double b = __builtin_bit_cast(double, ((unsigned long long)(unsigned)rh[1] << 32) | (unsigned)rl[1]);
    return a + b;
}

__device__ __forceinline__ void split_pair_f16(float a, float b, unsigned& hi, unsigned& lo) {
    unsigned h;
    float la, lb;
    asm("v_cvt_pk_f16_f32 %0, %1, %2" : "=v"(h) : "v"(a), "v"(b));
    asm("v_fma_mix_f32 %0, %1, -1.0, %2 op_sel:[0,0,0] op_sel_hi:[1,0,0]" : "=v"(la) : "v"(h), "v"(a));
    asm("v_fma_mix_f32 %0, %1, -1.0, %2 op_sel:[1,0,0] op_sel_hi:[1,0,0]" : "=v"(lb) : "v"(h), "v"(b));
    asm("v_cvt_pk_f16_f32 %0, %1, %2" : "=v"(lo) : "v"(la), "v"(lb));
    hi = h;
}

__device__ __forceinline__ double wave_sum_f64(double v) {
#define DPP_ADD64(ctrl_)                                                                                        \
    {                                                                                                           \
        const unsigned long long u_ = __builtin_bit_cast(unsigned long long, v);                                \
        const int lo_ = __builtin_amdgcn_update_dpp(0, (int)(unsigned)u_, ctrl_, 0xf, 0xf, false);             \
        const int hi_ = __builtin_amdgcn_update_dpp(0, (int)(unsigned)(u_ >> 32), ctrl_, 0xf, 0xf, false);     \
        v += __builtin_bit_cast(double, ((unsigned long long)(unsigned)hi_ << 32) | (unsigned long long)(unsigned)lo_); \
    }
    DPP_ADD64(0xB1)
    DPP_ADD64(0x4E)
    DPP_ADD64(0x141)
    DPP_ADD64(0x140)
#undef DPP_ADD64
    v = sum_xor16_f64(v);
    v = sum_xor32_f64(v);
    return v;
}

__device__ __forceinline__ double seg_sum_f64(double v, int seg) {
#define DPP_ADD64(ctrl_)                                                                                        \
    {                                                                                                           \
        const unsigned long long u_ = __builtin_bit_cast(unsigned long long, v);                                \
        const int lo_ = __builtin_amdgcn_update_dpp(0, (int)(unsigned)u_, ctrl_, 0xf, 0xf, false);             \
        const int hi_ = __builtin_amdgcn_update_dpp(0, (int)(unsigned)(u_ >> 32), ctrl_, 0xf, 0xf, false);     \
        v += __builtin_bit_cast(double, ((unsigned long long)(unsigned)hi_ << 32) | (unsigned long long)(unsigned)lo_); \
    }
    if (seg > 1) DPP_ADD64(0xB1)
    if (seg > 2) DPP_ADD64(0x4E)
    if (seg > 4) DPP_ADD64(0x141)
    if (seg > 8) DPP_ADD64(0x140)
#undef DPP_ADD64
    if (seg > 16) v = sum_xor16_f64(v);
    if (seg > 32) v = sum_xor32_f64(v);
    return v;
}

__device__ __forceinline__ void sample_mean_rstd_wave(const StatsRef& st, int b, int lane, float& mean, float& rstd) {
    const long long r0 = (long long)b * st.HW;
    const int first = (int)(r0 / st.m_tile);
    const int last = (int)((r0 + st.HW - 1) / st.m_tile);
    const int n = (last - first + 1) * st.n_tiles;
    if (n <= 8) {
        sample_mean_rstd(st, b, mean, rstd);
        return;
    }
    const double* p = st.p + (size_t)b * st.slots * 2;
    double s1 = 0.0, s2 = 0.0;
    for (int i = lane; i < n; i += 64) { s1 += p[2 * i]; s2 += p[2 * i + 1]; }
    s1 = wave_sum_f64(s1);
    s2 = wave_sum_f64(s2);
    const double m = s1 * st.inv_count;
    double var = s2 * st.inv_count - m * m;
    if (var < 0.0) var = 0.0;
    mean = (float)m;
    rstd = (float)(1.0 / sqrt(var + 1e-5));
}

__device__ __forceinline__ void film_coef_row_wave(const FilmSpec& f, int b, int lane, float* dst) {
    const int C = f.C;
    const int t = (f.temb != nullptr) ? f.t_dev[f.t_count == 1 ? 0 : b] : 0;
    float mean = 0.f, rstd = 1.f;
    if (f.st.p != nullptr) sample_mean_rstd_wave(f.st, b, lane, mean, rstd);
    for (int c = lane; c < C; c += 64) {
        float sc = 1.f, be = 0.f;
        if (f.st.p != nullptr) { sc = rstd * f.gamma[c]; be = f.beta[c] - mean * sc; }
        if (f.temb != nullptr) be += f.temb[(size_t)t * C + c];
        float fs = 1.f, fb = 0.f;
        if (f.film != nullptr) { fs = f.film[(size_t)b * 2 * C + c]; fb = f.film[(size_t)b * 2 * C + C + c]; }
        dst[c] = fs * sc;
        dst[C + c] = fs * be + fb;
    }
}

__device__ __forceinline__ float row16_sum_dpp(float v) {
#define DPP_ADD(ctrl_)                                                                                          \
    v += __builtin_bit_cast(float, __builtin_amdgcn_update_dpp(0, __builtin_bit_cast(int, v), ctrl_, 0xf, 0xf, false));
    DPP_ADD(0xB1)
    DPP_ADD(0x4E)
    DPP_ADD(0x141)
    DPP_ADD(0x140)
#undef DPP_ADD
    return v;
}

__device__ __forceinline__ float erf_bf(float x) {
    const float t = fabsf(x);
    const float p = t * t;
    float r = __builtin_bit_cast(float, 0xba1345e1u) * p + __builtin_bit_cast(float, 0x3ba10414u);
    r = r * p + __builtin_bit_cast(float, 0xbcdac9b8u);
    r = r * p + __builtin_bit_cast(float, 0x3de703beu);
    r = r * p + __builtin_bit_cast(float, 0xbec09330u);
    r = r * p + __builtin_bit_cast(float, 0x3e0375d0u);
    const float small = t * r + t;
    float q = t * __builtin_bit_cast(float, 0x378e98abu) + __builtin_bit_cast(float, 0xb9c68948u);
    q = t * q + __builtin_bit_cast(float, 0x3b7cd369u);
    q = t * q + __builtin_bit_cast(float, 0xbcc618b2u);
    q = t * q + __builtin_bit_cast(float, 0x3dda74e4u);
    q = t * q + __builtin_bit_cast(float, 0x3f228afdu);
    q = t * q + __builtin_bit_cast(float, 0x3e03c728u);
    q = t * q + t;
    const float a = -q * 1.44269504f;
    const float al = __fmaf_rn(-q, 1.44269504f, -a) - q * 1.925963033e-8f;
    const float e = __builtin_amdgcn_exp2f(a) * (1.0f + al * 0.69314718f);
    const float large = 1.0f - e;
    const float m = (t < 1.0f) ? small : large;
    return copysignf(m, x);
}

__device__ __forceinline__ float gelu_erf(float v) {
    const float z = fabsf(v);
    const float t = __builtin_amdgcn_rcpf(__fmaf_rn(0.3275911f * 0.70710678118654752440f, z, 1.0f));
    float p = __fmaf_rn(0.5f * 1.061405429f, t, 0.5f * -1.453152027f);
    p = __fmaf_rn(p, t, 0.5f * 1.421413741f);
    p = __fmaf_rn(p, t, 0.5f * -0.284496736f);
    p = __fmaf_rn(p, t, 0.5f * 0.254829592f);
    const float e = __builtin_amdgcn_exp2f(v * v * -0.72134752044448170368f);
    const float q = (p * t) * e;
    return __fmaf_rn(-z, q, fmaxf(v, 0.f));
}

__device__ __forceinline__ float wave_sum(float v) {
#pragma unroll
    for (int o = 32; o > 0; o >>= 1) v += __shfl_xor(v, o, 64);
    return v;
}
__device__ __forceinline__ float half_sum(float v) {
#pragma unroll
    for (int o = 16; o > 0; o >>= 1) v += __shfl_xor(v, o, 64);
    return v;
}

}
```

state_policy_diffusionmodel_amd/csrc/kernels.h:

```cpp
#pragma once
#include <hip/hip_runtime.h>
#include <stdint.h>
#include <mutex>
#include <set>
#include <utility>
#include <vector>

namespace spdm {

inline hipError_t allow_full_lds(const void* kern) {
    static std::mutex mu;
    static std::set<std::pair<int, const void*>> done;
    int dev = 0;
    hipError_t e = hipGetDevice(&dev);
    if (e != hipSuccess) return e;
    std::lock_guard<std::mutex> lk(mu);
    if (done.count({dev, kern})) return hipSuccess;
    e = hipFuncSetAttribute(kern, hipFuncAttributeMaxDynamicSharedMemorySize, (int)(160 * 1024));
    if (e == hipSuccess) done.insert({dev, kern});
    return e;
}

struct StatsRef {
    const double* p;
    int slots;
    int m_tile;
    int n_tiles;
    int HW;
    double inv_count;
};

__host__ __device__ inline int stats_slots(int HW, int m_tile, int n_tiles) {
    return ((HW + m_tile - 2) / m_tile + 1) * n_tiles;
}

enum : unsigned {
    SW_NO_WIDE = 1u << 0, SW_NO_WIDE128 = 1u << 1, SW_NO_W2 = 1u << 2, SW_NO_T512 = 1u << 3, SW_T512 = 1u << 4,
    SW_T3_BIG = 1u << 5, SW_NO_SMALL_TPI3 = 1u << 6, SW_WIDE_N64_2X2 = 1u << 7, SW_NO_SA_FUSED = 1u << 8,
    SW_NO_SA_TAIL = 1u << 9, SW_ATTN_VALU = 1u << 10, SW_SA_NO_WLDS = 1u << 11, SW_NO_FILM_FOLD = 1u << 12,
    SW_NO_GRAPH = 1u << 13, SW_NO_SPLITK = 1u << 14, SW_ARENA_TRACE = 1u << 15, SW_NO_WIDE_PIPE = 1u << 16, SW_NO_SKINNY = 1u << 17, SW_DEEP = 1u << 18,
    SW_NO_FILM_LOCAL = 1u << 19, SW_NO_FUSED_SRC = 1u << 20, SW_FILM_LOCAL = 1u << 21, SW_PIN_GEOMETRY = 1u << 22, SW_NO_WP4 = 1u << 23, SW_G2 = 1u << 24, SW_NO_WP8 = 1u << 25, SW_NO_SA_HEAD = 1u << 26, SW_SA_HEAD = 1u << 27, SW_NO_REG64 = 1u << 28,
    SW_NO_SA_CROP = 1u << 29, SW_NO_SA_OUTC = 1u << 30,
};
struct SwitchName { const char* env; unsigned bit; };
inline const SwitchName* switch_table(int* n) {
    static const SwitchName t[] = {
        {"SPDM_NO_WIDE", SW_NO_WIDE}, {"SPDM_NO_WIDE128", SW_NO_WIDE128}, {"SPDM_NO_W2", SW_NO_W2}, {"SPDM_NO_T512", SW_NO_T512},
        {"SPDM_T512", SW_T512}, {"SPDM_T3_BIG", SW_T3_BIG}, {"SPDM_NO_SMALL_TPI3", SW_NO_SMALL_TPI3},
        {"SPDM_WIDE_N64_2X2", SW_WIDE_N64_2X2}, {"SPDM_NO_SA_FUSED", SW_NO_SA_FUSED}, {"SPDM_NO_SA_TAIL", SW_NO_SA_TAIL},
        {"SPDM_ATTN_VALU", SW_ATTN_VALU}, {"SPDM_SA_NO_WLDS", SW_SA_NO_WLDS}, {"SPDM_NO_FILM_FOLD", SW_NO_FILM_FOLD},
        {"SPDM_NO_GRAPH", SW_NO_GRAPH}, {"SPDM_NO_SPLITK", SW_NO_SPLITK}, {"SPDM_ARENA_TRACE", SW_ARENA_TRACE}, {"SPDM_NO_WIDE_PIPE", SW_NO_WIDE_PIPE}, {"SPDM_NO_SKINNY", SW_NO_SKINNY}, {"SPDM_DEEP", SW_DEEP},
        {"SPDM_NO_FILM_LOCAL", SW_NO_FILM_LOCAL}, {"SPDM_NO_FUSED_SRC", SW_NO_FUSED_SRC},
        {"SPDM_FILM_LOCAL", SW_FILM_LOCAL}, {"SPDM_PIN_GEOMETRY", SW_PIN_GEOMETRY},
        {"SPDM_NO_WP4", SW_NO_WP4}, {"SPDM_G2", SW_G2}, {"SPDM_NO_WP8", SW_NO_WP8},
        {"SPDM_NO_SA_HEAD", SW_NO_SA_HEAD}, {"SPDM_SA_HEAD", SW_SA_HEAD}, {"SPDM_NO_REG64", SW_NO_REG64},
        {"SPDM_NO_SA_CROP", SW_NO_SA_CROP}, {"SPDM_NO_SA_OUTC", SW_NO_SA_OUTC}};
    *n = (int)(sizeof(t) / sizeof(t[0]));
    return t;
}
unsigned switches_from_env();
int spdm_tune(int idx, int dflt);

enum { PRO_NONE = 0, PRO_GN = 1, PRO_GN_GELU = 2, PRO_POOL = 3, PRO_UPCAT = 4 };
enum { EPI_STATS = 0, EPI_BIAS = 1, EPI_BIAS_GELU = 2, EPI_BIAS_RESID = 3, EPI_PLAIN = 4 };

enum { ROUTE_GEMM = 0, ROUTE_SKINNY = 1, ROUTE_REG = 2, ROUTE_WIDE = 3 };
enum { VAR_PLAIN = 0, VAR_W2 = 1, VAR_WP4 = 2, VAR_WP8 = 3, VAR_PIPE = 4, VAR_G2 = 5 };
struct GemmRoute { int kernel, variant, m_tile, n_tile; };

struct GemmArgs {
    const float* src;  int src_ld;
    const float* wgt;
    int split;
    const float* wgt_frag;
    float* dst;        int dst_ld;
    int M, K, N;
    int geom_M;
    int taps;
    int H, W, HW;
    int pro;  StatsRef pro_stats;  const float* pro_gamma;  const float* pro_beta;
    int up_C;  const float* skip;  int skip_ld;  StatsRef skip_stats;  const float* skip_gamma;  const float* skip_beta;
    int epi;  double* epi_stats;   const float* bias;  const float* resid;  int resid_ld;
    double* row_stats;
    int ksplit;  float* partial;
    unsigned sw;
    int debug;
    unsigned long long* stamps;
    GemmRoute* route;
};
enum { DBG_NO_MFMA = 1, DBG_NO_WLOAD = 2, DBG_NO_GELU = 4, DBG_NO_STORE = 8, DBG_NO_ALOAD = 16, DBG_PP = 64, DBG_STAMP = 128 };

struct GemmGeom {
    int m_tile, n_tile, n_tiles;
    int slots;
    int ksplit;
    int skinny;
    int reg;
    int st_m_tile, st_n_tiles;
};
GemmGeom gemm_geometry(int M, int N, int K, int HW, int W, int taps, int split, unsigned sw, bool stats_epi = false);
GemmGeom gemm_geometry(const GemmArgs& a);
constexpr size_t SPLITK_WORKSPACE_BYTES = (size_t)48 << 20;
__host__ __device__ inline int combine_rows(int HW, int N) {
    int r = HW;
    while ((r & 1) == 0 && (long long)r * N > 2048) r >>= 1;
    return r;
}
bool conv_skinny_geometry(int M, int N, int K, int HW, int W, int taps, int split, unsigned sw, int* m_tile, int* n_tile);
hipError_t launch_conv_skinny(const GemmArgs& a, const GemmGeom& g, hipStream_t s);
bool conv_reg_geometry(int M, int N, int K, int HW, int W, int taps, int split, unsigned sw);
hipError_t launch_conv_reg64(const GemmArgs& a, const GemmGeom& g, hipStream_t s);
hipError_t launch_splitk_combine(const float* partial, int ksplit, float* dst, int M, int N, int HW, double* stats,
                                 hipStream_t s);
hipError_t launch_gemm(const GemmArgs& a, hipStream_t s);
bool gemm_takes_fused_source(const GemmArgs& a);
bool gemm_takes_two_sources(const GemmArgs& a);
double gemm_flops(const GemmArgs& a);
bool conv_wide_supported(const GemmArgs& a, const GemmGeom& g);
hipError_t launch_conv_wide(const GemmArgs& a, const GemmGeom& g, hipStream_t s);

int conv_in_parts(int Hp, int Wp, int B);
hipError_t launch_conv_in(const float* x, const float* w , float* dst, double* stats,
                          int B, int H0, int D, int Hp, int Wp, int lh, int lw, int* step_dev, int* t_dev,
                          const int* timesteps_dev, int n_steps, int adv, hipStream_t s, int B_geom = 0);

struct AffineSrc {
    const float* x; int C;
    StatsRef st; const float* gamma; const float* beta;
};
hipError_t launch_pool(const AffineSrc& src, float* dst, int B, int H, int W, hipStream_t s);
hipError_t launch_upcat(const AffineSrc& up, const AffineSrc& skip, float* dst, int B, int Hin, int Win,
                        hipStream_t s);
hipError_t launch_film_apply(const AffineSrc& src, const float* temb_table , const int* t_dev,
                             int t_count, const float* film , float* dst, double* row_stats,
                             int B, int HW, hipStream_t s);
struct FilmSpec {
    StatsRef st; const float* gamma; const float* beta;
    const float* temb; const int* t_dev; int t_count;
    const float* film;
    int C;
    int on;
};
hipError_t launch_film_coef(const AffineSrc& src, const float* temb_table, const int* t_dev, int t_count, const float* film,
                            float* ab, int B, hipStream_t s);
hipError_t launch_encoder_convs(const float* img, const float* w1, const float* b1, const float* w2, const float* b2,
                                const float* w3, const float* b3, float* feat, int n_images, hipStream_t s);
hipError_t launch_encoder_train_convs(const float* img, const float* w1, const float* b1, const float* w2, const float* b2,
                                      const float* w3, const float* b3, float* feat, float* x3, int n_images, hipStream_t s);
hipError_t launch_encoder_kinks(const float* img, const float* w1, const float* b1, const float* w2, const float* b2,
                                const float* w3, const float* b3, float* feat, float* x3, int n_images, hipStream_t s);
hipError_t launch_encoder_x2(const float* img, const float* w1, const float* b1, int n_images, float* x2, hipStream_t s);
hipError_t launch_encoder_dz3(const float* dfeat, const float* feat, int n_images, float* dz3, hipStream_t s);
hipError_t launch_encoder_dz2(const float* dx3, const float* x3, int n_images, float* dz2, hipStream_t s);
int encoder_conv1_wgrad_blocks(int n_images);
hipError_t launch_encoder_conv1_wgrad(const float* img, const float* dx2, const float* x2, int n_images, float* part,
                                      float* dw, float* db, hipStream_t s);
hipError_t launch_add(const float* src, size_t n, float* dst, hipStream_t s);
hipError_t launch_decoder_convs(const float* h0, const float* w2, const float* b2, const float* w4, const float* b4,
                                const float* w6, const float* b6, float* recon, int n_frames, hipStream_t s);
hipError_t launch_decoder_train_convs(const float* h0, const float* w2, const float* b2, const float* w4, const float* b4,
                                      const float* w6, const float* b6, float* recon, const float* target, float* a1, float* a2,
                                      double* sq, int n_frames, hipStream_t s);
hipError_t launch_decoder_kinks(const float* latent, const float* w0, const float* b0, const float* w2, const float* b2,
                                const float* w4, const float* b4, float* a1, float* a2, int n_frames, hipStream_t s);
hipError_t launch_decoder_loss(const double* sq, int n_frames, float* loss, hipStream_t s);
hipError_t launch_decoder_bwd6(const float* recon, const float* target, const float* a2, const float* w6, float scale,
                               int n_frames, float* dz4, float* part, float* dw, float* db, hipStream_t s);
hipError_t launch_decoder_dgrad4(const float* dz4, const float* a1, const float* w4, int n_frames, float* dz2, hipStream_t s);
int decoder_colsum_slab_rows(long long M);
int decoder_colsum_slabs(long long M);
hipError_t launch_decoder_colsum(const float* src, int C, long long M, int n_out, int fold, float* part, float* dst, hipStream_t s);
hipError_t launch_decoder_unperm_conv(const float* src, int cin, int cout, float* dst, hipStream_t s);
hipError_t launch_decoder_unperm_linear(const float* src, float* dst, hipStream_t s);
hipError_t launch_gn_apply(const AffineSrc& src, float* dst, int B, int HW, hipStream_t s);
hipError_t launch_layernorm(const float* x, const float* g, const float* b, float* y, int rows, int C,
                            hipStream_t s);
hipError_t launch_mish_pad(const float* cond, float* dst, int B, int cond_dim, int Kp, hipStream_t s);
hipError_t launch_silu(const float* x, float* y, size_t n, hipStream_t s);
hipError_t launch_gelu(const float* x, float* y, size_t n, hipStream_t s);
hipError_t launch_silu_pad(const float* cond, float* dst, int B, int cond_dim, int Kp, hipStream_t s);
hipError_t launch_dc_finish(const AffineSrc& src, const float* res, float* dst, int B, int HW, hipStream_t s);
hipError_t launch_simple_tail(const AffineSrc& src, int Cr, const float* temb, int temb_ld, const int* t_dev, int t_count,
                              const float* cemb, int cemb_ld, float* dst, int Co, int B, int HW, hipStream_t s);

struct StepArgs {
    const float* feat;
    const float* w; float bias;
    float* x;
    float* eps_out;
    const float* eps_in;
    const float* coef;
    const int* step_dev;
    int kind;
    const float* noise;
    const unsigned long long* rng_dev;
    int* flag_dev;
    const float* inpaint; int inp_h; int inpaint_per_sample;
    float* history;
    const void* const* ptrs_dev;
    int B, H0, D, Hp, Wp, lh, lw;
};
hipError_t launch_out_step(const StepArgs& a, hipStream_t s);

int wgrad_chunks(long long M, int taps, int Co, int Ci, size_t budget_floats);
hipError_t launch_wgrad(const float* dy, int ldy, const float* x, int ldx, long long M, int H, int W, int taps, int Co, int Ci,
                        int conv9, float* partial, size_t budget_floats, float* dst, hipStream_t s);
hipError_t launch_wgrad_mapped(const float* dy, const float* x, long long M, int H, int W, int taps, int Co, int Ci,
                               const int* pos_o, int no, const int* pos_i, int ni, float* partial, size_t budget_floats, float* dst,
                               hipStream_t s);
hipError_t launch_colsum(const float* src, int ld, long long M, int C, float* dst, hipStream_t s);
hipError_t launch_gn_stats(const float* y, int B, int n, float* mean, float* rstd, hipStream_t s);
hipError_t launch_gn_stats_real(const float* y, int B, int n, int cnt, float* mean, float* rstd, hipStream_t s);
hipError_t launch_gn_act(const float* y, const float* mean, const float* rstd, const float* gamma, const float* beta, int B,
                         int HW, int C, int gelu, float* out, hipStream_t s);
hipError_t launch_gn_bwd(const float* y, const float* mean, const float* rstd, const float* gamma, const float* beta,
                         const float* g, int gelu, int B, int HW, int C, float* dy, float* dgb, hipStream_t s);
hipError_t launch_gn_param(const float* p0, const float* p1, int B, int C, float* dgamma, float* dbeta, hipStream_t s);
hipError_t launch_film_bwd(const float* z, const float* temb, const int* t_dev, int t_count, const float* film,
                           const float* dout, int B, int HW, int C, float* dz, float* de, float* dfilm, hipStream_t s);
hipError_t launch_gather_rows(const float* table, const int* t_dev, int t_count, int B, int n, float* out, hipStream_t s);
hipError_t launch_pad(const float* x, int B, int H0, int D, int Hp, int Wp, int lh, int lw, float* xp, hipStream_t s);
hipError_t launch_conv_in_plain(const float* xp, const float* w , int B, int H, int W, float* out, hipStream_t s);
hipError_t launch_outc(const float* u, const float* w, float bias, long long M, float* out, hipStream_t s);
hipError_t launch_outc_bwd(const float* deps, const float* w, long long M, float* du, hipStream_t s);
hipError_t launch_mse(const float* eps_pad, const float* noise, int B, int H0, int D, int Hp, int Wp, int lh, int lw,
                      float* loss, float* deps_pad, float* eps_out, hipStream_t s);
hipError_t launch_pool_bwd(const float* in, const float* dout, int B, int H, int W, int C, float* din, hipStream_t s);
hipError_t launch_up_bwd(const float* dcat, int ld, int B, int h, int w, int C, float* dx, hipStream_t s);
hipError_t launch_add_cols(const float* src, int ld, int c0, long long M, int C, float* dst, hipStream_t s);
hipError_t launch_mish_bwd(const float* dm, int nblk, int B, int ld, const float* cond, int cond_dim, float* grad_cond,
                           hipStream_t s);

hipError_t launch_ln_fwd(const float* x, const float* g, const float* b, long long rows, int C, float* y, float* mean, float* rstd,
                         hipStream_t s);
constexpr int LN_BWD_ROWS = 64;
int ln_bwd_blocks(long long rows);
hipError_t launch_ln_bwd(const float* x, const float* mean, const float* rstd, const float* gamma, const float* gy,
                         const float* add, long long rows, int C, float* dx, float* part, hipStream_t s);
hipError_t launch_gelu_bwd(const float* u, const float* dh, size_t n, float* du, hipStream_t s);

hipError_t launch_gn_bwd_mapped(const float* y, const float* mean, const float* rstd, const float* gamma, const float* beta,
                                const float* g, int gelu, int B, int HW, int C, const int* pos, int nreal, float* dy, float* dgb,
                                hipStream_t s);
hipError_t launch_gn_param_mapped(const float* p0, const float* p1, int B, int C, const int* pos, int nreal, float* dgamma,
                                  float* dbeta, hipStream_t s);
hipError_t launch_gn_res(const float* y, const float* mean, const float* rstd, const float* gamma, const float* beta,
                         const float* res, int B, int HW, int C, float* pre, float* out, hipStream_t s);
hipError_t launch_simple_tail_fwd(const float* y, const float* mean, const float* rstd, const float* gamma, const float* beta,
                                  int Cz, int Cr, const float* temb, int temb_ld, const float* cemb, int cemb_ld, int B, int HW,
                                  int Co, float* out, hipStream_t s);
hipError_t launch_simple_tail_bwd(const float* dout, int B, int HW, int Co, int Cr, int Cz, float* dz, float* dtemb, float* dcemb,
                                  int cemb_ld, hipStream_t s);
hipError_t launch_time_rows_scaled(const float* pe, const int* t_dev, int t_count, const float* scale, int B, int n, float* out,
                                   hipStream_t s);
hipError_t launch_silu_bwd(const float* ds, int ld, const float* cond, int B, int cond_dim, float* grad_cond, hipStream_t s);
bool attn_train_supported(int L, int C, int heads);
hipError_t launch_attn_fwd_lse(const float* qkv, float* out, float* lse, int B, int L, int C, int heads, hipStream_t s);
hipError_t launch_attn_bwd(const float* qkv, const float* out, const float* dout, const float* lse, float* dqkv, int B, int L,
                           int C, int heads, hipStream_t s);

constexpr int ADAM_GRID = 1024;
constexpr int OPTIM_MAX_SEGMENTS = 4;
struct OptimSeg { float* p; const float* g; float* m; float* v; unsigned long long n; };
struct OptimArgs {
    OptimSeg seg[OPTIM_MAX_SEGMENTS];
    int nseg;
    int clip;
    float max_norm;
    float beta1, beta1_lo, one_minus_beta1, beta2, beta2_lo, one_minus_beta2, eps;
    float step_size;
    float bc2_sqrt;
    unsigned long long quads, per;
};
hipError_t launch_adam_step(OptimArgs a, double* workspace, hipStream_t s);

hipError_t launch_advance(int* step_dev, int* t_dev, const int* timesteps_dev, int n_steps, hipStream_t s);
hipError_t launch_set_step(int* step_dev, int* t_dev, const int* timesteps_dev, int n_steps, int i, hipStream_t s);

hipError_t launch_attention(const float* qkv , float* out , int B, int L, int C,
                            int heads, hipStream_t s);
hipError_t launch_attention_auto(const float* qkv, float* out, int B, int L, int C, int heads, unsigned sw, hipStream_t s);

bool sa_fused_supported(int L, int C);
struct SaCrop { int H0, D, Wp, lh, lw; const float* outc_w; float outc_b; float* eps; };
bool sa_crop_supported(int L, int C, int H0, int D);
hipError_t launch_sa_fused64(const float* x, float* out, int B, int L, const float* ln1_g, const float* ln1_b,
                             const float* ln2_g, const float* ln2_b, const void* const w_hl[8], const float* bqkv,
                             const float* bo, const float* b1, const float* b2, const float* ab, unsigned sw, hipStream_t s,
                             const FilmSpec* fs = nullptr, const SaCrop* crop = nullptr);

bool sa_tail_supported(int C, unsigned sw);
hipError_t launch_sa_tail(int C, const float* o, const float* x, float* out, int rows, const float* wf_o, const float* wf_1,
                          const float* wf_2, const float* b_o, const float* b_1, const float* b_2, const float* ln_g,
                          const float* ln_b, const float* ab, int L, hipStream_t s, const FilmSpec* fs = nullptr);
bool sa_tail_film_local(int C, int L);
bool sa_head_supported(int C, int L, unsigned sw);
hipError_t launch_sa_head(int C, const float* x, float* att, int rows, const float* wf_in, const float* b_in, const float* ln_g,
                          const float* ln_b, const float* ab, int L, hipStream_t s, const FilmSpec* fs = nullptr);
hipError_t launch_sa_qkv(int C, const float* x, float* qkv, int rows, const float* wf_in, const float* b_in, const float* ln_g,
                         const float* ln_b, const float* ab, int L, hipStream_t s, const FilmSpec* fs = nullptr);

enum { WL_F32 = 0, WL_SPLIT, WL_FRAG, WL_PERM_HI, WL_PERM_LO, WL_RANGE, WL_NFMT };
struct WeightCopy {
    long long src = 0;
    long long stride[3] = {0, 0, 0};
    int n[3] = {1, 1, 1};
    int lim[3] = {1, 1, 1};
    int tab[3] = {-1, -1, -1};
    int fmt = WL_F32;
    int taps = 1, N = 0, K = 0;
    int slot = -1;
    void* dst = nullptr;
    long long count = 0;
    long long blk0 = 0;
};
long long weight_copy_blocks(long long count);
hipError_t launch_weight_copies(int fmt, const float* blob, const long long* tabs, const WeightCopy* copies, int n_copies,
                                long long blocks, int* flags, hipStream_t s);

}
```

state_policy_diffusionmodel_amd/csrc/spdm_api.hip:

```cpp
#include <hip/hip_runtime.h>

#include <algorithm>
#include <cmath>
#include <cstdarg>
#include <cstdio>
#include <cstdlib>
#include <cstring>
#include <map>
#include <set>
#include <string>
#include <vector>

#include "../../include/spdm.h"
#include "kernels.h"

using namespace spdm;

static thread_local char g_err[512] = "";
static int fail(int code, const char* fmt, ...) {
    va_list ap;
    va_start(ap, fmt);
    vsnprintf(g_err, sizeof(g_err), fmt, ap);
    va_end(ap);
    return code;
// ... 2935 lines not shown
    double* sv_sq = nullptr;
    int sv_cap = 0, sv_n = 0;
    float *bw_dz4 = nullptr, *bw_dz2 = nullptr, *bw_dh0 = nullptr;
    int bw_cap = 0;
    float *wg_part = nullptr, *wg_tmp = nullptr, *cs_part = nullptr, *w6_part = nullptr, *g_tmp = nullptr;
};
static constexpr int DEC_FEAT = 64 * 12 * 12, DEC_LATENT = 128, DEC_PIX = 3 * 96 * 96;
static constexpr int DEC_A1 = 576 * 32, DEC_A2 = 2304 * 16;
static constexpr size_t DEC_WG_FLOATS = (size_t)8 * DEC_LATENT * DEC_FEAT;
static constexpr size_t DEC_WG_SLABS = 256;

static const struct { const char* name; std::vector<int> shape; } DEC_ITEMS[8] = {
    {"0.weight", {DEC_FEAT, DEC_LATENT}}, {"0.bias", {DEC_FEAT}}, {"2.weight", {64, 32, 2, 2}}, {"2.bias", {32}},
    {"4.weight", {32, 16, 2, 2}}, {"4.bias", {16}}, {"6.weight", {16, 3, 2, 2}}, {"6.bias", {3}}};

static WeightCopy convt_copy(long long src, int cin, int cout) {
    WeightCopy c = Recorder::dense(src, cin, 4, cout);
    c.stride[0] = (long long)cout * 4; c.stride[1] = 1; c.stride[2] = 4;
    return c;
}

extern "C" void spdm_decoder_destroy(spdm_decoder* d) {
    if (!d) return;
    (void)hipSetDevice(d->device);
    for (void* p : d->owned) (void)hipFree(p);
    delete d;
}

extern "C" int spdm_decoder_create(int32_t device, const float* blob, size_t n, const spdm_tensor_index* index, int32_t n_index,
                                   spdm_decoder** out) {
    if (!blob || !index || n_index <= 0 || !out) return fail(SPDM_ERR_INVALID, "null argument");
    HIP_TRY(hipSetDevice(device));
    spdm_decoder* d = new spdm_decoder();
    d->device = device;
    d->blob_floats = n;
    Recorder R(d->wt, n, index, n_index);
    R.plan = false;
    bool ok = true;
    for (int k = 0; k < 8 && ok; ++k) {
        const long long off = R.at(DEC_ITEMS[k].name, DEC_ITEMS[k].shape);
        if (off < 0) { ok = false; break; }
        d->off[k] = off;
        d->numel[k] = 1;
        for (int v : DEC_ITEMS[k].shape) d->numel[k] *= (size_t)v;
    }
    if (ok) {
        WeightCopy w0 = Recorder::dense(d->off[0], 144, 64, DEC_LATENT);
        w0.stride[0] = DEC_LATENT; w0.stride[1] = (long long)144 * DEC_LATENT; w0.stride[2] = 1;
        WeightCopy b0 = Recorder::dense(d->off[1], 1, 144, 64);
        b0.stride[1] = 1; b0.stride[2] = 144;
        d->w0 = R.f32(w0);
        d->b0 = R.f32(b0);
        d->w2 = R.f32(convt_copy(d->off[2], 64, 32));
        d->b2 = R.f32(Recorder::dense(d->off[3], 1, 1, 32));
        d->w4 = R.f32(convt_copy(d->off[4], 32, 16));
        d->b4 = R.f32(Recorder::dense(d->off[5], 1, 1, 16));
        d->w6 = R.f32(convt_copy(d->off[6], 16, 3));
        d->b6 = R.f32(Recorder::dense(d->off[7], 1, 1, 3));
    }
    DevBlob db;
    int rc = R.err;
    if (rc == SPDM_OK) rc = db.upload(blob, n);
    if (rc == SPDM_OK) rc = R.finish(db.p);
    if (rc != SPDM_OK) {
        spdm_decoder_destroy(d);
        return rc == SPDM_ERR_MISSING ? SPDM_ERR_INVALID : rc;
    }
    *out = d;
    return SPDM_OK;
}

static int dec_alloc(spdm_decoder* d, float** p, size_t floats) {
    void* q = nullptr;
    if (hipMalloc(&q, floats * sizeof(float)) != hipSuccess) return fail(SPDM_ERR_NOMEM, "decoder workspace (%zu floats)", floats);
    d->owned.push_back(q);
    *p = (float*)q;
    return SPDM_OK;
}
static void dec_release(spdm_decoder* d, float** p) {
    if (!*p) return;
    for (auto it = d->owned.begin(); it != d->owned.end(); ++it)
        if (*it == (void*)*p) { d->owned.erase(it); break; }
    (void)hipFree(*p);
    *p = nullptr;
}
static int dec_linear(spdm_decoder* d, const float* latent, int m, float* h0, hipStream_t s) {
    const LinW lin{d->w0, nullptr, d->b0, DEC_LATENT, DEC_FEAT};
    HIP_TRY(launch_gemm(linear_args(AffineSrc{latent, DEC_LATENT}, m, 0, lin, false, 0, EPI_BIAS, h0), s));
    return SPDM_OK;
}

extern "C" int spdm_decoder_forward(spdm_decoder* d, int32_t n, const float* d_latent, float* d_recon, void* stream) {
    if (!d || !d_latent || !d_recon || n <= 0) return fail(SPDM_ERR_INVALID, "bad argument");
    HIP_TRY(hipSetDevice(d->device));
    hipStream_t s = (hipStream_t)stream;
    const int chunk = std::min<int>(n, ENC_CHUNK);
    if (d->chunk < chunk) {
        SPDM_TRY(dec_alloc(d, &d->h0, (size_t)chunk * DEC_FEAT));
        d->chunk = chunk;
    }
    for (int i0 = 0; i0 < n; i0 += chunk) {
        const int m = std::min(chunk, n - i0);
        SPDM_TRY(dec_linear(d, d_latent + (size_t)i0 * DEC_LATENT, m, d->h0, s));
        HIP_TRY(launch_decoder_convs(d->h0, d->w2, d->b2, d->w4, d->b4, d->w6, d->b6, d_recon + (size_t)i0 * DEC_PIX, m, s));
    }
    if (!stream) HIP_TRY(hipStreamSynchronize(s));
    return SPDM_OK;
}

extern "C" int spdm_decoder_train_loss(spdm_decoder* d, int32_t n, const float* d_latent, const float* d_target, float* d_recon,
                                       float* d_loss, void* stream) {
    if (!d || !d_latent || !d_target || !d_loss || n <= 0) return fail(SPDM_ERR_INVALID, "bad argument");
    HIP_TRY(hipSetDevice(d->device));
    hipStream_t s = (hipStream_t)stream;
    d->sv_n = 0;
    if (!d->w0g) {
        SPDM_TRY(dec_alloc(d, &d->wg_part, DEC_WG_FLOATS));
        SPDM_TRY(dec_alloc(d, &d->wg_tmp, (size_t)DEC_FEAT * DEC_LATENT));
        SPDM_TRY(dec_alloc(d, &d->cs_part, (size_t)decoder_colsum_slabs(ENC_CHUNK) * DEC_FEAT));
        SPDM_TRY(dec_alloc(d, &d->w6_part, (size_t)ENC_CHUNK * 208));
        SPDM_TRY(dec_alloc(d, &d->g_tmp, d->blob_floats));
        Recorder R(d->wt, d->blob_floats);
        R.plan = false;
        WeightCopy g = Recorder::dense(d->off[0], DEC_LATENT, 144, 64);
        g.stride[0] = 1; g.stride[1] = DEC_LATENT; g.stride[2] = (long long)144 * DEC_LATENT;
        float* const w0g = R.f32(g);
        SPDM_TRY(R.err);
        SPDM_TRY(d->wt.upload(false));
        float* const T = d->g_tmp;
        HIP_TRY(launch_decoder_unperm_linear(d->w0, T + d->off[0], s));
        HIP_TRY(launch_decoder_colsum(d->b0, DEC_FEAT, 1, DEC_FEAT, 1, d->cs_part, T + d->off[1], s));
        HIP_TRY(launch_decoder_unperm_conv(d->w2, 64, 32, T + d->off[2], s));
        HIP_TRY(launch_decoder_unperm_conv(d->w4, 32, 16, T + d->off[4], s));
        HIP_TRY(launch_decoder_unperm_conv(d->w6, 16, 3, T + d->off[6], s));
        const float* const bias[3] = {d->b2, d->b4, d->b6};
        for (int k = 0; k < 3; ++k)
            HIP_TRY(hipMemcpyAsync(T + d->off[3 + 2 * k], bias[k], d->numel[3 + 2 * k] * sizeof(float), hipMemcpyDeviceToDevice, s));
        SPDM_TRY(d->wt.relayout(T, s));
        d->w0g = w0g;
    }
    if (d->sv_cap < n) {
        HIP_TRY(hipDeviceSynchronize());
        dec_release(d, &d->sv_h0); dec_release(d, &d->sv_a1); dec_release(d, &d->sv_a2); dec_release(d, &d->sv_recon);
        dec_release(d, (float**)&d->sv_sq);
        d->sv_cap = 0;
        SPDM_TRY(dec_alloc(d, &d->sv_h0, (size_t)n * DEC_FEAT));
        SPDM_TRY(dec_alloc(d, &d->sv_a1, (size_t)n * DEC_A1));
        SPDM_TRY(dec_alloc(d, &d->sv_a2, (size_t)n * DEC_A2));
        SPDM_TRY(dec_alloc(d, &d->sv_recon, (size_t)n * DEC_PIX));
        SPDM_TRY(dec_alloc(d, (float**)&d->sv_sq, (size_t)n * 2));
        d->sv_cap = n;
    }
    const int chunk = std::min<int>(n, ENC_CHUNK);
    for (int i0 = 0; i0 < n; i0 += chunk) {
        const int m = std::min(chunk, n - i0);
        float* h0 = d->sv_h0 + (size_t)i0 * DEC_FEAT;
        SPDM_TRY(dec_linear(d, d_latent + (size_t)i0 * DEC_LATENT, m, h0, s));
        HIP_TRY(launch_decoder_train_convs(h0, d->w2, d->b2, d->w4, d->b4, d->w6, d->b6, d->sv_recon + (size_t)i0 * DEC_PIX,
                                           d_target + (size_t)i0 * DEC_PIX, d->sv_a1 + (size_t)i0 * DEC_A1,
                                           d->sv_a2 + (size_t)i0 * DEC_A2, d->sv_sq + i0, m, s));
        HIP_TRY(launch_decoder_kinks(d_latent + (size_t)i0 * DEC_LATENT, d->w0, d->b0, d->w2, d->b2, d->w4, d->b4,
                                     d->sv_a1 + (size_t)i0 * DEC_A1, d->sv_a2 + (size_t)i0 * DEC_A2, m, s));
    }
    HIP_TRY(launch_decoder_loss(d->sv_sq, n, d_loss, s));
    if (d_recon) HIP_TRY(hipMemcpyAsync(d_recon, d->sv_recon, (size_t)n * DEC_PIX * sizeof(float), hipMemcpyDeviceToDevice, s));
    d->sv_n = n;
    if (!stream) HIP_TRY(hipStreamSynchronize(s));
    return SPDM_OK;
}

extern "C" int spdm_decoder_backward(spdm_decoder* d, int32_t n, const float* d_latent, const float* d_target, float* d_grad,
                                     float* d_grad_latent, void* stream) {
    if (!d || !d_latent || !d_target || !d_grad || !d_grad_latent || n <= 0) return fail(SPDM_ERR_INVALID, "bad argument");
    if (d->sv_n == 0) return fail(SPDM_ERR_STATE, "decoder_backward: no spdm_decoder_train_loss is pending");
    if (d->sv_n != n) return fail(SPDM_ERR_STATE, "decoder_backward: %d frames, the pending train_loss had %d", n, d->sv_n);
    HIP_TRY(hipSetDevice(d->device));
    hipStream_t s = (hipStream_t)stream;
    const int chunk = std::min<int>(n, ENC_CHUNK);
    if (d->bw_cap < chunk) {
        HIP_TRY(hipDeviceSynchronize());
        dec_release(d, &d->bw_dz4); dec_release(d, &d->bw_dz2); dec_release(d, &d->bw_dh0);
        d->bw_cap = 0;
        SPDM_TRY(dec_alloc(d, &d->bw_dz4, (size_t)chunk * DEC_A2));
        SPDM_TRY(dec_alloc(d, &d->bw_dz2, (size_t)chunk * DEC_A1));
        SPDM_TRY(dec_alloc(d, &d->bw_dh0, (size_t)chunk * DEC_FEAT));
        d->bw_cap = chunk;
    }
    d->sv_n = 0;
    const float scale = (float)(2.0 / ((double)n * DEC_PIX));
    HIP_TRY(hipMemsetAsync(d_grad, 0, d->blob_floats * sizeof(float), s));
    for (int i0 = 0; i0 < n; i0 += chunk) {
        const int m = std::min(chunk, n - i0);
        float* G = i0 == 0 ? d_grad : d->g_tmp;
        const float* lat = d_latent + (size_t)i0 * DEC_LATENT;
        const float* h0 = d->sv_h0 + (size_t)i0 * DEC_FEAT;
        const float* a1 = d->sv_a1 + (size_t)i0 * DEC_A1;
        const float* a2 = d->sv_a2 + (size_t)i0 * DEC_A2;
        const long long M1 = (long long)m * 144, M2 = (long long)m * 576;
        HIP_TRY(launch_decoder_bwd6(d->sv_recon + (size_t)i0 * DEC_PIX, d_target + (size_t)i0 * DEC_PIX, a2, d->w6, scale, m,
                                    d->bw_dz4, d->w6_part, G + d->off[6], G + d->off[7], s));
        HIP_TRY(launch_wgrad(a1, 32, d->bw_dz4, 64, M2, 1, 1, 1, 32, 64, 0, d->wg_part, DEC_WG_SLABS * 32 * 64, d->wg_tmp, s));
        HIP_TRY(launch_decoder_unperm_conv(d->wg_tmp, 32, 16, G + d->off[4], s));
        HIP_TRY(launch_decoder_colsum(d->bw_dz4, 64, M2, 16, 4, d->cs_part, G + d->off[5], s));
        HIP_TRY(launch_decoder_dgrad4(d->bw_dz4, a1, d->w4, m, d->bw_dz2, s));
        HIP_TRY(launch_wgrad(h0, 64, d->bw_dz2, 128, M1, 1, 1, 1, 64, 128, 0, d->wg_part, DEC_WG_SLABS * 64 * 128, d->wg_tmp, s));
        HIP_TRY(launch_decoder_unperm_conv(d->wg_tmp, 64, 32, G + d->off[2], s));
        HIP_TRY(launch_decoder_colsum(d->bw_dz2, 128, M1, 32, 4, d->cs_part, G + d->off[3], s));
        HIP_TRY(launch_gemm(gemm_args((int)M1, 0, 1, 1, 128, 64, 1, 0, 0, nullptr, PRO_NONE, AffineSrc{d->bw_dz2, 128}, 0, AffineSrc{},
                                      d->w2, nullptr, d->bw_dh0, 64, EPI_PLAIN, nullptr), s));
        HIP_TRY(launch_wgrad(d->bw_dh0, DEC_FEAT, lat, DEC_LATENT, m, 1, 1, 1, DEC_FEAT, DEC_LATENT, 0, d->wg_part, DEC_WG_FLOATS,
                             d->wg_tmp, s));
        HIP_TRY(launch_decoder_unperm_linear(d->wg_tmp, G + d->off[0], s));
        HIP_TRY(launch_decoder_colsum(d->bw_dh0, DEC_FEAT, m, DEC_FEAT, 1, d->cs_part, G + d->off[1], s));
        HIP_TRY(launch_gemm(gemm_args(m, 0, 1, 1, DEC_FEAT, DEC_LATENT, 1, 0, 0, nullptr, PRO_NONE, AffineSrc{d->bw_dh0, DEC_FEAT}, 0,
                                      AffineSrc{}, d->w0g, nullptr, d_grad_latent + (size_t)i0 * DEC_LATENT, DEC_LATENT, EPI_PLAIN,
                                      nullptr), s));
        if (i0 != 0) {
            for (int k = 0; k < 8; ++k) HIP_TRY(launch_add(d->g_tmp + d->off[k], d->numel[k], d_grad + d->off[k], s));
        }
    }
    if (!stream) HIP_TRY(hipStreamSynchronize(s));
    return SPDM_OK;
}

extern "C" int spdm_decoder_update_weights(spdm_decoder* d, const float* d_blob, size_t n, void* stream) {
    if (!d || !d_blob) return fail(SPDM_ERR_INVALID, "null argument");
    if (n != d->blob_floats) return fail(SPDM_ERR_INVALID, "blob has %zu floats; the one given to spdm_decoder_create had %zu", n, d->blob_floats);
    HIP_TRY(hipSetDevice(d->device));
    hipStream_t s = (hipStream_t)stream;
    d->sv_n = 0;
    SPDM_TRY(d->wt.relayout(d_blob, s));
    if (!stream) HIP_TRY(hipStreamSynchronize(s));
    return SPDM_OK;
}

extern "C" size_t spdm_adam_workspace_doubles(void) { return (size_t)ADAM_GRID + 1; }
extern "C" size_t spdm_adam_norm_index(void) { return (size_t)ADAM_GRID; }

static double beta_as_written(float b) {
    char buf[40];
    for (int prec = 1; prec <= 9; ++prec) {
        snprintf(buf, sizeof(buf), "%.*g", prec, (double)b);
        const double d = strtod(buf, nullptr);
        if ((float)d == b) return d;
    }
    return (double)b;
}

extern "C" int spdm_adam_step(int32_t device, const spdm_optim_segment* h_segments, int32_t n_segments, int64_t step, float lr,
                              float beta1, float beta2, float eps, float max_norm, double* d_workspace, void* stream) {
    if (!h_segments || !d_workspace) return fail(SPDM_ERR_INVALID, "adam_step: null argument");
    if (n_segments < 1 || n_segments > SPDM_OPTIM_MAX_SEGMENTS)
        return fail(SPDM_ERR_INVALID, "adam_step: %d segments (1 .. %d)", n_segments, SPDM_OPTIM_MAX_SEGMENTS);
    if (step < 1) return fail(SPDM_ERR_INVALID, "adam_step: step %lld (the count including this step, >= 1)", (long long)step);
    if (!std::isfinite(lr) || !std::isfinite(eps) || !std::isfinite(beta1) || !std::isfinite(beta2))
        return fail(SPDM_ERR_INVALID, "adam_step: lr, eps and the betas must be finite");
    if (!(beta1 >= 0.f && beta1 < 1.f) || !(beta2 >= 0.f && beta2 < 1.f))
        return fail(SPDM_ERR_INVALID, "adam_step: betas (%g, %g) outside [0, 1)", (double)beta1, (double)beta2);
    if (std::isnan(max_norm)) return fail(SPDM_ERR_INVALID, "adam_step: max_norm is NaN");
    if ((uintptr_t)d_workspace % 16) return fail(SPDM_ERR_INVALID, "adam_step: d_workspace is not 16-byte aligned");
    OptimArgs a = {};
    for (int i = 0; i < n_segments; ++i) {
        const spdm_optim_segment& g = h_segments[i];
        if (!g.d_param || !g.d_grad || !g.d_exp_avg || !g.d_exp_avg_sq) return fail(SPDM_ERR_INVALID, "adam_step: segment %d: null pointer", i);
        if (g.numel == 0) return fail(SPDM_ERR_INVALID, "adam_step: segment %d is empty", i);
        if (((uintptr_t)g.d_param | (uintptr_t)g.d_grad | (uintptr_t)g.d_exp_avg | (uintptr_t)g.d_exp_avg_sq) % 16)
            return fail(SPDM_ERR_INVALID, "adam_step: segment %d: a pointer is not 16-byte aligned", i);
        a.seg[i] = {g.d_param, g.d_grad, g.d_exp_avg, g.d_exp_avg_sq, (unsigned long long)g.numel};
    }
    const double b1 = beta_as_written(beta1), b2 = beta_as_written(beta2);
    const double bc1 = 1.0 - std::pow(b1, (double)step), bc2 = 1.0 - std::pow(b2, (double)step);
    a.nseg = n_segments;
    a.clip = max_norm > 0.f;
    a.max_norm = max_norm;
    a.beta1 = (float)b1;  a.beta1_lo = (float)(b1 - (double)a.beta1);  a.one_minus_beta1 = (float)(1.0 - b1);
    a.beta2 = (float)b2;  a.beta2_lo = (float)(b2 - (double)a.beta2);  a.one_minus_beta2 = (float)(1.0 - b2);
    a.eps = eps;
    a.step_size = (float)((double)lr / bc1);
    a.bc2_sqrt = (float)std::sqrt(bc2);
    HIP_TRY(hipSetDevice(device));
    HIP_TRY(launch_adam_step(a, d_workspace, (hipStream_t)stream));
    if (!stream) HIP_TRY(hipStreamSynchronize(nullptr));
    return SPDM_OK;
}

extern "C" int spdm_debug_geometry(int32_t M, int32_t N, int32_t K, int32_t HW, int32_t W, int32_t taps, uint32_t switches,
                                   int32_t out[10]) {
    if (!out || M <= 0 || N <= 0 || K <= 0 || HW <= 0 || W <= 0 || M % HW != 0) return fail(SPDM_ERR_INVALID, "bad argument");
    const GemmGeom g = gemm_geometry(M, N, K, HW, W, taps, 1, switches, true);
    out[0] = g.m_tile; out[1] = g.n_tile; out[2] = g.n_tiles; out[3] = g.slots; out[4] = g.ksplit; out[5] = g.skinny | (g.reg << 1);
    out[6] = g.st_m_tile; out[7] = g.st_n_tiles;
    out[8] = stats_slots_reserved(HW, N, g.slots);
    out[9] = combine_rows(HW, N);
    return SPDM_OK;
}

extern "C" int spdm_op_gelu(const float* d_x, float* d_y, size_t n, void* stream) {
    if (!d_x || !d_y || n == 0) return fail(SPDM_ERR_INVALID, "bad argument");
    HIP_TRY(launch_gelu(d_x, d_y, n, (hipStream_t)stream));
    if (!stream) HIP_TRY(hipStreamSynchronize(nullptr));
    return SPDM_OK;
}

extern "C" int spdm_op_gemm(spdm_op_gemm_args* p) {
    if (!p) return fail(SPDM_ERR_INVALID, "op_gemm: null argument");
    spdm_op_gemm_args& q = *p;
    for (int i = 0; i < 10; ++i) q.out[i] = -1;
    const int HW = q.H * q.W;
    if (q.B <= 0 || q.H <= 0 || q.W <= 0 || q.K <= 0 || q.N <= 0) return fail(SPDM_ERR_INVALID, "op_gemm: empty shape");
    if (!(q.taps == 9 || q.taps == 3 || q.taps == 1)) return fail(SPDM_ERR_INVALID, "op_gemm: taps must be 9, 3 or 1");
    if (q.taps == 3 && q.W != 1) return fail(SPDM_ERR_INVALID, "op_gemm: 3-tap convolutions need W == 1");
    if (q.taps == 1 && HW != 1) return fail(SPDM_ERR_INVALID, "op_gemm: a Linear layer has H == W == 1 (B = rows)");
    if (q.taps != 1 && q.W > 8) return fail(SPDM_ERR_INVALID, "op_gemm: maps wider than 8");
    if (q.K % 32 != 0 || q.N % 64 != 0) return fail(SPDM_ERR_INVALID, "op_gemm: K %% 32 == 0 and N %% 64 == 0 required (K %d, N %d)", q.K, q.N);
    if (q.pro < PRO_NONE || q.pro > PRO_UPCAT || q.epi < EPI_STATS || q.epi > EPI_PLAIN) return fail(SPDM_ERR_INVALID, "op_gemm: unknown pro / epi");
    if (!q.d_src || !q.d_dst || !q.h_weight) return fail(SPDM_ERR_INVALID, "op_gemm: src, dst and weight are required");
    if (q.dst_ld < q.N || q.dst_ld % 4 || q.src_ld % 4) return fail(SPDM_ERR_INVALID, "op_gemm: bad leading dimension");
    const bool fused = q.pro == PRO_POOL || q.pro == PRO_UPCAT, two = !fused && q.d_skip != nullptr;
    if (q.src_ld < ((fused && q.pro == PRO_UPCAT) || two ? q.up_C : q.K)) return fail(SPDM_ERR_INVALID, "op_gemm: src_ld too small");
    if ((q.d_skip != nullptr) != (q.pro == PRO_UPCAT || two)) return fail(SPDM_ERR_INVALID, "op_gemm: skip is the second source of pro 4 / a two-source input only");
    if (q.d_skip && (q.up_C <= 0 || q.up_C >= q.K || q.skip_ld % 4 || q.skip_ld < q.K - q.up_C)) return fail(SPDM_ERR_INVALID, "op_gemm: bad up_C / skip_ld");
    if (two && (q.pro != PRO_NONE || q.d_src_stats)) return fail(SPDM_ERR_INVALID, "op_gemm: a two-source input takes its prologue from the skip statistics only");
    if (q.d_skip_stats && !q.d_skip) return fail(SPDM_ERR_INVALID, "op_gemm: skip statistics without skip");
    if ((q.pro == PRO_GN || q.pro == PRO_GN_GELU) && !q.d_src_stats) return fail(SPDM_ERR_INVALID, "op_gemm: GroupNorm prologue without statistics");
    if ((q.d_src_stats && (!q.d_gamma || !q.d_beta || q.src_slots <= 0 || q.src_m_tile <= 0 || q.src_n_tiles <= 0)) ||
        (q.d_skip_stats && (!q.d_skip_gamma || !q.d_skip_beta || q.skip_slots <= 0 || q.skip_m_tile <= 0 || q.skip_n_tiles <= 0)))
        return fail(SPDM_ERR_INVALID, "op_gemm: pending GroupNorm needs gamma, beta and the partials' geometry");
    if (q.d_src_stats && q.pro == PRO_NONE) return fail(SPDM_ERR_INVALID, "op_gemm: src statistics given with pro 0");
    if (q.epi != EPI_STATS && q.epi != EPI_PLAIN && !q.d_bias) return fail(SPDM_ERR_INVALID, "op_gemm: bias epilogue without bias");
    if (q.epi == EPI_BIAS_RESID && (!q.d_resid || q.resid_ld < q.N || q.resid_ld % 4)) return fail(SPDM_ERR_INVALID, "op_gemm: bad residual");
    if (q.d_row_stats && q.taps != 1) return fail(SPDM_ERR_INVALID, "op_gemm: row statistics are a Linear layer's output");
    const int M = q.B * HW;
    const int src_rows = q.pro == PRO_POOL ? 4 * HW : q.pro == PRO_UPCAT ? HW / 4 : HW;
    if (q.pro == PRO_UPCAT && ((q.H & 1) || (q.W & 1))) return fail(SPDM_ERR_INVALID, "op_gemm: upsample read-through needs an even map");
    const int split = q.split ? 1 : 0;
    DevBlob db;
    WeightTable wt;
    Recorder R(wt, (size_t)q.N * q.K * (q.taps == 1 ? 1 : 9));
    float *dw = nullptr, *dwf = nullptr;
    auto walk = [&]() {
        const WeightCopy v = q.taps == 1 ? Recorder::dense(0, 1, q.N, q.K) : Recorder::conv_taps(0, q.N, q.K, q.taps);
        dw = split ? R.split(v, q.K, "weight") : R.f32(v);
        dwf = (split && dw && q.taps != 1) ? R.frag(v, q.taps, q.N, q.K) : nullptr;
        return R.err;
    };
    SPDM_TRY(db.upload(q.h_weight, R.n));
    SPDM_TRY(R.both_passes(db.p, walk));
    if (!dw) return fail(SPDM_ERR_INVALID, "op_gemm: weights outside the split format's range (the loader keeps such a layer on the exact path)");
    const unsigned sw = switches_from_env();
    const bool may_partial = split && q.taps != 1 && q.epi == EPI_STATS && !(sw & SW_NO_SPLITK);
    const GemmGeom g = gemm_geometry(M, q.N, q.K, HW, q.W, q.taps, split, sw, may_partial);
    if (q.epi == EPI_STATS && (!q.d_stats || q.stats_cap < (size_t)q.B * g.slots * 2))
        return fail(SPDM_ERR_INVALID, "op_gemm: statistics buffer needs %zu doubles", (size_t)q.B * g.slots * 2);
    if (q.d_row_stats && q.row_stats_cap < (size_t)M * g.n_tiles * 2)
        return fail(SPDM_ERR_INVALID, "op_gemm: row statistics buffer needs %zu doubles", (size_t)M * g.n_tiles * 2);
    if (g.ksplit > 1 && (size_t)g.ksplit * M * q.N * sizeof(float) > SPLITK_WORKSPACE_BYTES)
        return fail(SPDM_ERR_INVALID, "op_gemm: split-K slabs exceed the workspace");
    float* dp = nullptr;
    if (may_partial) SPDM_TRY(wt.alloc((void**)&dp, g.ksplit > 1 ? (size_t)g.ksplit * M * q.N * sizeof(float) : 0));
    auto ref = [](const double* st, int slots, int m_tile, int n_tiles, int rows, int cnorm) {
        return StatsRef{st, slots, m_tile, n_tiles, rows, 1.0 / ((double)cnorm * rows)};
    };
    const int src_c = (q.pro == PRO_UPCAT || two) ? q.up_C : q.K;
    AffineSrc src{q.d_src, q.src_ld}, skip{q.d_skip, q.skip_ld};
    if (q.d_src_stats)
        src = AffineSrc{q.d_src, q.src_ld, ref(q.d_src_stats, q.src_slots, q.src_m_tile, q.src_n_tiles, src_rows,
                                               q.src_cnorm > 0 ? q.src_cnorm : src_c), q.d_gamma, q.d_beta};
    if (q.d_skip_stats)
        skip = AffineSrc{q.d_skip, q.skip_ld, ref(q.d_skip_stats, q.skip_slots, q.skip_m_tile, q.skip_n_tiles, HW,
                                                  q.skip_cnorm > 0 ? q.skip_cnorm : q.K - q.up_C), q.d_skip_gamma, q.d_skip_beta};
    const int pro = (two && q.d_skip_stats) ? PRO_GN : q.pro;
    GemmArgs a = gemm_args(M, M, q.H, q.W, q.K, q.N, q.taps, split, sw, dp, pro, src, q.up_C, skip, dw,
                           dwf, q.d_dst, q.dst_ld, q.epi, q.epi == EPI_STATS ? q.d_stats : nullptr, q.d_bias,
                           q.d_resid, q.resid_ld, q.d_row_stats);
    if (fused && !gemm_takes_fused_source(a))
        return fail(SPDM_ERR_INVALID, "op_gemm: this launch does not take a fused source (the plan materialises it)");
    if (two && !gemm_takes_two_sources(a))
        return fail(SPDM_ERR_INVALID, "op_gemm: this launch does not take a two-source input (the plan concatenates)");
    GemmRoute r{-1, -1, -1, -1};
    a.route = &r;
    if (q.epi == EPI_STATS) HIP_TRY(hipMemset(q.d_stats, 0xff, (size_t)q.B * g.slots * 2 * sizeof(double)));
    if (q.d_row_stats) HIP_TRY(hipMemset(q.d_row_stats, 0xff, (size_t)M * g.n_tiles * 2 * sizeof(double)));
    const hipError_t el = launch_gemm(a, nullptr);
    const hipError_t es = hipDeviceSynchronize();
    if (el != hipSuccess)
        return fail(el == hipErrorInvalidValue && r.kernel < 0 ? SPDM_ERR_INVALID : SPDM_ERR_HIP,
                    "op_gemm: launch_gemm failed (%s) %s; device: %s", hipGetErrorString(el),
                    r.kernel < 0 ? "before any kernel was dispatched (a host-side shape contract)" : "after a kernel was dispatched",
                    hipGetErrorString(es));
    if (es != hipSuccess) return fail(SPDM_ERR_HIP, "op_gemm: %s", hipGetErrorString(es));
    q.out[0] = r.kernel; q.out[1] = r.variant; q.out[2] = r.m_tile; q.out[3] = r.n_tile; q.out[4] = g.ksplit;
    q.out[5] = two ? 1 : 0; q.out[6] = fused ? 1 : 0; q.out[7] = g.slots; q.out[8] = g.st_m_tile; q.out[9] = g.st_n_tiles;
    return SPDM_OK;
}
```

Baseline: 496,900.

## Add whole-sample tile staging to wide conv kernels and cheaper GELU

Adds a template mode to the wide 3x3 conv kernel for tiles that hold whole samples. In that mode the halo rows, clamp and validity masking are dropped, the per-row sample index becomes a shift, and when a tile is exactly one sample the group-norm mean and rstd are read once into scalars. A selector dispatches these variants when the shape allows, and a switch can turn it off. GELU is also replaced with a polynomial-in-exp2 approximation clamped at 6. The risks are more template instantiations and a small change in GELU accuracy.

```diff
diff --git a/include/spdm.h b/include/spdm.h
--- a/include/spdm.h
+++ b/include/spdm.h
@@ -154,6 +154,8 @@
 int  spdm_debug_geometry(int32_t M, int32_t N, int32_t K, int32_t HW, int32_t W, int32_t taps, uint32_t switches,
                          int32_t out[10]);
 
+int  spdm_debug_whole_tiles(void);
+
 int  spdm_op_gelu(const float* d_x, float* d_y, size_t n, void* stream);
 
 typedef struct {
diff --git a/state_policy_diffusionmodel_amd/_lib.py b/state_policy_diffusionmodel_amd/_lib.py
--- a/state_policy_diffusionmodel_amd/_lib.py
+++ b/state_policy_diffusionmodel_amd/_lib.py
@@ -95,6 +95,7 @@
     "spdm_op_gelu": (c_int32, [c_void_p, c_void_p, c_size_t, c_void_p]),
     "spdm_op_gemm": (c_int32, [POINTER(SpdmOpGemmArgs)]),
     "spdm_debug_geometry": (c_int32, [c_int32] * 6 + [ctypes.c_uint32, POINTER(c_int32 * 10)]),
+    "spdm_debug_whole_tiles": (c_int32, []),
     "spdm_bench_gemm": (c_int32, [c_int32] * 12 + [POINTER(c_double)]),
 }
 
diff --git a/state_policy_diffusionmodel_amd/csrc/conv_wide.hip b/state_policy_diffusionmodel_amd/csrc/conv_wide.hip
--- a/state_policy_diffusionmodel_amd/csrc/conv_wide.hip
+++ b/state_policy_diffusionmodel_amd/csrc/conv_wide.hip
@@ -53,7 +53,7 @@
     return f32x2{__builtin_bit_cast(float, h), __builtin_bit_cast(float, l)};
 }
 
-template <int NT, int PRO, bool W2, int RT, int WN, bool PIPE, bool TWO = false, int WP = 0, bool G2 = false>
+template <int NT, int PRO, bool W2, int RT, int WN, bool PIPE, bool TWO = false, int WP = 0, bool G2 = false, int WH = 0>
 #ifndef WIDE_MINB
 #define WIDE_MINB 2
 #endif
@@ -64,7 +64,9 @@
     constexpr int NTHR = 256;
     constexpr int RP = NTHR / 8;
     constexpr int M_T = WM * RW, N_T = WN * NT * 32;
-    constexpr int APASS = (M_T + 18 + RP - 1) / RP;
+    constexpr bool WHOLE = (WH != 0);
+    constexpr bool ONE = (WH == 2);
+    constexpr int APASS = WHOLE ? M_T / RP : (M_T + 18 + RP - 1) / RP;
     constexpr int FAR = (W2 || WP) ? 4 : 3;
     constexpr int FBR = (NT == 2) ? 2 : 3;
     constexpr int PH = 3 * NT;
@@ -81,13 +83,14 @@
     constexpr bool WP8 = (WP == 8);
     constexpr int NI8 = (M_T + 18 + 6) / 8 + 1;
     static_assert(!G2 || (NT == 2 && RT == 4 && !W2 && !PIPE && !WP && !WIDE_DB), "two chunks per hand-over: the plain tap loop, 64 rows per wave");
+    static_assert(!WHOLE || (!G2 && !WIDE_DB && !WIDE_EARLY), "whole-sample staging: not in the hand-over experiments");
     extern __shared__ __attribute__((aligned(16))) float smem[];
 
     const int tid = threadIdx.x, lane = tid & 63;
     const int wave = __builtin_amdgcn_readfirstlane(tid >> 6);
     const int wm = wave / WN, wn = wave % WN, l16 = lane & 15, kg = lane >> 4;
     const int HW = a.HW, W = a.W, H = a.H, M = a.M, K = a.K, N = a.N;
-    const int halo = W + 1;
+    const int halo = WHOLE ? 0 : W + 1;
     const int QA = M_T + 2 * halo;
     const int QZ = WP8 ? 8 * NI8 + 2 : QA + 2;
 
@@ -133,7 +136,13 @@
     constexpr bool pro = (PRO != PRO_NONE);
     constexpr bool pro_gelu = (PRO == PRO_GN_GELU);
     int bh_first = 0;
-    if (pro) {
+    float mu1 = 0.f, rs1 = 1.f;
+    const int lhw = WHOLE ? __builtin_ctz((unsigned)HW) : 0;
+    if constexpr (pro && ONE) {
+        sample_mean_rstd(a.pro_stats, m0 / HW, mu1, rs1);
+        mu1 = __builtin_bit_cast(float, __builtin_amdgcn_readfirstlane(__builtin_bit_cast(int, mu1)));
+        rs1 = __builtin_bit_cast(float, __builtin_amdgcn_readfirstlane(__builtin_bit_cast(int, rs1)));
+    } else if (pro) {
         const int lo = max(m0 - halo, 0), hi = min(m0 + M_T + halo, M) - 1;
         bh_first = lo / HW;
         const int bh_last = hi / HW;
@@ -150,7 +159,7 @@
     unsigned avalid = 0u;
     unsigned long long abidx = 0ull;
 #pragma unroll
-    for (int p = 0; p < APASS; ++p) {
+    for (int p = 0; p < (WHOLE ? 0 : APASS); ++p) {
         const int q = p * RP + srow_t;
         const int m = m0 - halo + q;
         const bool v = (q < QA) && (m >= 0) && (m < M);
@@ -167,7 +176,7 @@
 #define WIDE_ROWOFF(rt_) (W2 ? (((rt_) >> 1) * 32 + ((rt_) & 1)) : WP8 ? (rt_) : WP ? (((rt_) >> 2) * 64 + ((rt_) & 3)) : (rt_) * 16)
 #define WIDE_LDSOFF(rt_) (WP8 ? (rt_) * NI8 : WIDE_ROWOFF(rt_))
     const int rowlane = W2 ? 2 * l16 : WP ? WP * l16 : PERM ? (l16 < 4 ? l16 : l16 < 12 ? l16 + 4 : l16 - 8) : l16;
-    const int aoff0 = WP8 ? (2 + wm * 16 + l16) * LDK + kg * 4 : (wm * RW + rowlane + halo) * LDK + kg * 4;
+    const int aoff0 = WP8 ? ((WHOLE ? 0 : 2) + wm * 16 + l16) * LDK + kg * 4 : (wm * RW + rowlane + halo) * LDK + kg * 4;
     const int zoff = zrow * LDK + kg * 4;
     unsigned am[(RT + 2) / 3] = {};
 #pragma unroll
@@ -215,7 +224,7 @@
         const float* ab_ = (first_ ? abase : abase1) + cc_ * CK;                                     \
         const int ld_ = first_ ? a.src_ld : a.skip_ld;                                               \
         _Pragma("unroll") for (int p_ = 0; p_ < APASS; ++p_) {                                      \
-            const int mc_ = min(max(m0 - halo + p_ * RP + srow_o, 0), M - 1);                        \
+            const int mc_ = WHOLE ? m0 + p_ * RP + srow_o : min(max(m0 - halo + p_ * RP + srow_o, 0), M - 1); \
             areg_[p_] = *reinterpret_cast<const f32x4*>(ab_ + (size_t)mc_ * ld_);                     \
         }                                                                                            \
         if (pro) {                                                                                   \
@@ -223,30 +232,39 @@
             g4r_ = *reinterpret_cast<const f32x4*>(a.pro_gamma + cc_ * CK + c4 * 4);                  \
             b4r_ = *reinterpret_cast<const f32x4*>(a.pro_beta + cc_ * CK + c4 * 4);                   \
             if (TWO && first_) { g4r_ = f32x4{1.f, 1.f, 1.f, 1.f}; b4r_ = f32x4{0.f, 0.f, 0.f, 0.f}; } \
+            else if (ONE) g4r_ = rs1 * g4r_;                           \
         }                                                                                            \
     }
 #define WIDE_STAGE_A_(areg_, g4r_, b4r_, ident_, dst_)                                                                             \
     {                                                                                                \
         _Pragma("unroll") for (int p_ = 0; p_ < APASS; ++p_) {                                      \
             f32x4 v_ = areg_[p_];                                                                     \
-            if (pro) {                                                                               \
-                const int bi_ = (int)((abidx >> (BB * p_)) & ((1ull << BB) - 1));                                  \
+            if (pro && ONE) {                                         \
+                const float mu_ = (TWO && ident_) ? 0.f : mu1;                                       \
+                v_.x = (v_.x - mu_) * g4r_.x + b4r_.x;                                                \
+                v_.y = (v_.y - mu_) * g4r_.y + b4r_.y;                                                \
+                v_.z = (v_.z - mu_) * g4r_.z + b4r_.z;                                                \
+                v_.w = (v_.w - mu_) * g4r_.w + b4r_.w;                                                \
+            } else if (pro) {                                                                        \
+                const int bi_ = WHOLE ? (p_ * RP + srow_o) >> lhw : (int)((abidx >> (BB * p_)) & ((1ull << BB) - 1)); \
                 float rs_ = srstd[bi_], mu_ = smean[bi_];                                            \
                 if (TWO && ident_) { rs_ = 1.f; mu_ = 0.f; }        \
                 v_.x = (v_.x - mu_) * (rs_ * g4r_.x) + b4r_.x;                                         \
                 v_.y = (v_.y - mu_) * (rs_ * g4r_.y) + b4r_.y;                                         \
                 v_.z = (v_.z - mu_) * (rs_ * g4r_.z) + b4r_.z;                                         \
                 v_.w = (v_.w - mu_) * (rs_ * g4r_.w) + b4r_.w;                                         \
+            }                                                                                        \
+            if (pro) {                                                                               \
                 if (pro_gelu) {                                                                      \
                     v_.x = gelu_erf(v_.x); v_.y = gelu_erf(v_.y);                                    \
                     v_.z = gelu_erf(v_.z); v_.w = gelu_erf(v_.w);                                    \
                 }                                                                                    \
             }                                                                                        \
-            if (!((avalid >> p_) & 1u)) v_ = f32x4{0.f, 0.f, 0.f, 0.f};                              \
+            if (!WHOLE && !((avalid >> p_) & 1u)) v_ = f32x4{0.f, 0.f, 0.f, 0.f};                       \
             const f32x2 p0_ = split2(v_.x, v_.y), p1_ = split2(v_.z, v_.w);                          \
             {                    \
                 const int q_ = p_ * RP + srow_o;                                                     \
-                float* row_ = (dst_) + (WP8 ? (q_ < QA ? ((q_ + 7) & 7) * NI8 + ((q_ + 7) >> 3) : 8 * NI8 + 1) : min(q_, QA + 1)) * LDK; \
+                float* row_ = (dst_) + (WHOLE ? (WP8 ? (q_ & 7) * NI8 + (q_ >> 3) : q_) : WP8 ? (q_ < QA ? ((q_ + 7) & 7) * NI8 + ((q_ + 7) >> 3) : 8 * NI8 + 1) : min(q_, QA + 1)) * LDK; \
                 *reinterpret_cast<f32x2*>(row_ + c4 * 2) = f32x2{p0_.x, p1_.x};              \
                 *reinterpret_cast<f32x2*>(row_ + 16 + c4 * 2) = f32x2{p0_.y, p1_.y};         \
             }                                                                                        \
@@ -377,32 +395,40 @@
             }
 #define PIPE_LOAD(slot_, chunk_, pass_)                                                              \
             {                                                                                        \
-                const int mc_ = min(max(pm0 + (pass_) * RP, 0), M - 1);                              \
+                const int mc_ = WHOLE ? pm0 + (pass_) * RP : min(max(pm0 + (pass_) * RP, 0), M - 1);    \
                 ar[slot_] = *reinterpret_cast<const f32x4*>(abase + (size_t)mc_ * a.src_ld + (chunk_) * CK); \
             }
 #define PIPE_GB(chunk_)                                                                              \
             if (pro) {                                                                               \
                 g4r = *reinterpret_cast<const f32x4*>(a.pro_gamma + (chunk_) * CK + c4 * 4);         \
                 b4r = *reinterpret_cast<const f32x4*>(a.pro_beta + (chunk_) * CK + c4 * 4);          \
+                if (ONE) g4r = rs1 * g4r;                                                            \
             }
 #define PIPE_STAGE(slot_, pass_)                                                                     \
             {                                                                                        \
                 f32x4 v_ = ar[slot_];                                                                \
-                if (pro) {                                                                           \
-                    const int bi_ = (int)((abidx >> (BB * (pass_))) & ((1ull << BB) - 1));           \
+                if (pro && ONE) {                                                                    \
+                    v_.x = (v_.x - mu1) * g4r.x + b4r.x;                                             \
+                    v_.y = (v_.y - mu1) * g4r.y + b4r.y;                                             \
+                    v_.z = (v_.z - mu1) * g4r.z + b4r.z;                                             \
+                    v_.w = (v_.w - mu1) * g4r.w + b4r.w;                                             \
+                } else if (pro) {                                                                    \
+                    const int bi_ = WHOLE ? ((pass_) * RP + srow_p) >> lhw : (int)((abidx >> (BB * (pass_))) & ((1ull << BB) - 1)); \
                     const float rs_ = srstd[bi_], mu_ = smean[bi_];                                  \
                     v_.x = (v_.x - mu_) * (rs_ * g4r.x) + b4r.x;                                     \
                     v_.y = (v_.y - mu_) * (rs_ * g4r.y) + b4r.y;                                     \
                     v_.z = (v_.z - mu_) * (rs_ * g4r.z) + b4r.z;                                     \
                     v_.w = (v_.w - mu_) * (rs_ * g4r.w) + b4r.w;                                     \
+                }                                                                                    \
+                if (pro) {                                                                           \
                     if (pro_gelu) {                                                                  \
                         v_.x = gelu_erf(v_.x); v_.y = gelu_erf(v_.y);                                \
                         v_.z = gelu_erf(v_.z); v_.w = gelu_erf(v_.w);                                \
                     }                                                                                \
                 }                                                                                    \
-                if (!((avalid >> (pass_)) & 1u)) v_ = f32x4{0.f, 0.f, 0.f, 0.f};                     \
+                if (!WHOLE && !((avalid >> (pass_)) & 1u)) v_ = f32x4{0.f, 0.f, 0.f, 0.f};              \
                 const f32x2 p0_ = split2(v_.x, v_.y), p1_ = split2(v_.z, v_.w);                      \
-                float* row_ = Awr + min((pass_) * RP + srow_p, QA + 1) * LDK;                        \
+                float* row_ = Awr + (WHOLE ? (pass_) * RP + srow_p : min((pass_) * RP + srow_p, QA + 1)) * LDK; \
                 *reinterpret_cast<f32x2*>(row_ + c4 * 2) = f32x2{p0_.x, p1_.x};                      \
                 *reinterpret_cast<f32x2*>(row_ + 16 + c4 * 2) = f32x2{p0_.y, p1_.y};                 \
             }
@@ -904,11 +930,12 @@
 #undef WIDE_ROWOFF
 }
 
-template <int NT, int PRO, bool W2 = false, int RT = 8, int WN = 2, bool PIPE = false, bool TWO = false, int WP = 0, bool G2 = false>
+template <int NT, int PRO, bool W2 = false, int RT = 8, int WN = 2, bool PIPE = false, bool TWO = false, int WP = 0, bool G2 = false, int WH = 0>
 hipError_t launch_wide_cfg(const GemmArgs& a, const GemmGeom& g, hipStream_t s) {
     constexpr int M_T = (4 / WN) * RT * 16, N_T = WN * 32 * NT, NTHR = 256;
-    constexpr int APASS = (M_T + 18 + 31) / 32, NSMAX = (APASS <= 9) ? 128 : (APASS <= 10) ? 64 : 32;
-    const int halo = a.W + 1;
+    constexpr int APASS = WH ? M_T / 32 : (M_T + 18 + 31) / 32, NSMAX = (APASS <= 9) ? 128 : (APASS <= 10) ? 64 : 32;
+    if (WH && (M_T % a.HW != 0 || a.M % M_T != 0 || (WH == 2 && a.HW != M_T))) return hipErrorInvalidValue;
+    const int halo = WH ? 0 : a.W + 1;
     const int QA = M_T + 2 * halo;
     const int NS = (((QA - 1) / a.HW + 2) + 3) & ~3;
     if (NS > NSMAX || g.m_tile != M_T || g.n_tile != N_T) return hipErrorInvalidValue;
@@ -920,13 +947,24 @@
     size_t lds = (size_t)(((DB || G2) ? 2 : 1) * QZ * LDK + 2 * NS) * sizeof(float);
     lds = std::max(lds, (size_t)((M_T / (W2 ? 2 : WP ? RT / 4 : WIDE_NH)) * N_T + (M_T / 4) * WN * 2) * sizeof(float));
     if (lds > 160 * 1024) return hipErrorInvalidValue;
-    auto kern = conv3x3_wide_kernel<NT, PRO, W2, RT, WN, PIPE, TWO, WP, G2>;
+    auto kern = conv3x3_wide_kernel<NT, PRO, W2, RT, WN, PIPE, TWO, WP, G2, WH>;
     if (hipError_t e = allow_full_lds(reinterpret_cast<const void*>(kern)); e != hipSuccess) return e;
     const int n_mtiles = (a.M + M_T - 1) / M_T;
     if (a.ksplit > 1 && a.K % 64 != 0) return hipErrorInvalidValue;
-    if (a.route) *a.route = GemmRoute{ROUTE_WIDE, WP == 4 ? VAR_WP4 : WP == 8 ? VAR_WP8 : W2 ? VAR_W2 : PIPE ? VAR_PIPE : G2 ? VAR_G2 : VAR_PLAIN, M_T, N_T};
+    if (a.route) *a.route = GemmRoute{ROUTE_WIDE, WP == 4 ? VAR_WP4 : WP == 8 ? VAR_WP8 : W2 ? VAR_W2 : PIPE ? VAR_PIPE : G2 ? VAR_G2 : VAR_PLAIN, M_T, N_T, WH};
     hipLaunchKernelGGL(kern, dim3(n_mtiles * g.n_tiles * std::max(a.ksplit, 1)), dim3(NTHR), lds, s, a, g.slots, NS);
     return hipGetLastError();
+}
+
+template <int MODES, int NT, int PRO, bool W2 = false, int RT = 8, int WN = 2, bool PIPE = false, bool TWO = false, int WP = 0>
+hipError_t launch_wide_sel(const GemmArgs& a, const GemmGeom& g, hipStream_t s) {
+    constexpr int M_T = (4 / WN) * RT * 16;
+    const bool whole = !(a.sw & SW_NO_WHOLE_TILES) && M_T % a.HW == 0 && a.M % M_T == 0;
+    if constexpr ((MODES & 2) != 0 && PRO != PRO_NONE)
+        if (whole && a.HW == M_T) return launch_wide_cfg<NT, PRO, W2, RT, WN, PIPE, TWO, WP, false, 2>(a, g, s);
+    if constexpr ((MODES & 1) != 0)
+        if (whole) return launch_wide_cfg<NT, PRO, W2, RT, WN, PIPE, TWO, WP, false, 1>(a, g, s);
+    return launch_wide_cfg<NT, PRO, W2, RT, WN, PIPE, TWO, WP, false, 0>(a, g, s);
 }
 
 }
@@ -961,38 +999,38 @@
         const bool two = a.skip != nullptr;
         if (g.m_tile == 128) {
             if (two) {
-                if (a.pro == PRO_NONE) return launch_wide_cfg<2, PRO_NONE, false, 4, 2, false, true, 4>(a, g, s);
-                return launch_wide_cfg<2, PRO_GN, false, 4, 2, false, true, 4>(a, g, s);
-            }
-            if (a.pro == PRO_NONE) return launch_wide_cfg<2, PRO_NONE, false, 4, 2, false, false, 4>(a, g, s);
-            if (a.pro == PRO_GN) return launch_wide_cfg<2, PRO_GN, false, 4, 2, false, false, 4>(a, g, s);
-            return launch_wide_cfg<2, PRO_GN_GELU, false, 4, 2, false, false, 4>(a, g, s);
+                if (a.pro == PRO_NONE) return launch_wide_sel<1, 2, PRO_NONE, false, 4, 2, false, true, 4>(a, g, s);
+                return launch_wide_sel<1, 2, PRO_GN, false, 4, 2, false, true, 4>(a, g, s);
+            }
+            if (a.pro == PRO_NONE) return launch_wide_sel<1, 2, PRO_NONE, false, 4, 2, false, false, 4>(a, g, s);
+            if (a.pro == PRO_GN) return launch_wide_sel<1, 2, PRO_GN, false, 4, 2, false, false, 4>(a, g, s);
+            return launch_wide_sel<1, 2, PRO_GN_GELU, false, 4, 2, false, false, 4>(a, g, s);
         }
         if (two) {
-            if (a.pro == PRO_NONE) return launch_wide_cfg<2, PRO_NONE, false, 8, 2, false, true, 4>(a, g, s);
-            return launch_wide_cfg<2, PRO_GN, false, 8, 2, false, true, 4>(a, g, s);
-        }
-        if (a.pro == PRO_NONE) return launch_wide_cfg<2, PRO_NONE, false, 8, 2, false, false, 4>(a, g, s);
-        if (a.pro == PRO_GN) return launch_wide_cfg<2, PRO_GN, false, 8, 2, false, false, 4>(a, g, s);
-        return launch_wide_cfg<2, PRO_GN_GELU, false, 8, 2, false, false, 4>(a, g, s);
+            if (a.pro == PRO_NONE) return launch_wide_sel<1, 2, PRO_NONE, false, 8, 2, false, true, 4>(a, g, s);
+            return launch_wide_sel<1, 2, PRO_GN, false, 8, 2, false, true, 4>(a, g, s);
+        }
+        if (a.pro == PRO_NONE) return launch_wide_sel<1, 2, PRO_NONE, false, 8, 2, false, false, 4>(a, g, s);
+        if (a.pro == PRO_GN) return launch_wide_sel<1, 2, PRO_GN, false, 8, 2, false, false, 4>(a, g, s);
+        return launch_wide_sel<1, 2, PRO_GN_GELU, false, 8, 2, false, false, 4>(a, g, s);
     }
     if (a.W == 8 && a.taps == 9 && g.n_tile == 128 && g.m_tile == 256 && a.HW % 32 == 0 && a.K % 64 == 0 && !(a.sw & SW_NO_WP8)) {
         if (a.skip != nullptr) {
-            if (a.pro == PRO_NONE) return launch_wide_cfg<2, PRO_NONE, false, 8, 2, false, true, 8>(a, g, s);
-            return launch_wide_cfg<2, PRO_GN, false, 8, 2, false, true, 8>(a, g, s);
-        }
-        if (a.pro == PRO_NONE) return launch_wide_cfg<2, PRO_NONE, false, 8, 2, false, false, 8>(a, g, s);
-        if (a.pro == PRO_GN) return launch_wide_cfg<2, PRO_GN, false, 8, 2, false, false, 8>(a, g, s);
-        return launch_wide_cfg<2, PRO_GN_GELU, false, 8, 2, false, false, 8>(a, g, s);
+            if (a.pro == PRO_NONE) return launch_wide_sel<3, 2, PRO_NONE, false, 8, 2, false, true, 8>(a, g, s);
+            return launch_wide_sel<3, 2, PRO_GN, false, 8, 2, false, true, 8>(a, g, s);
+        }
+        if (a.pro == PRO_NONE) return launch_wide_sel<3, 2, PRO_NONE, false, 8, 2, false, false, 8>(a, g, s);
+        if (a.pro == PRO_GN) return launch_wide_sel<3, 2, PRO_GN, false, 8, 2, false, false, 8>(a, g, s);
+        return launch_wide_sel<3, 2, PRO_GN_GELU, false, 8, 2, false, false, 8>(a, g, s);
     }
     if (a.skip != nullptr) {
         if (g.m_tile == 128) {
-            if (a.pro == PRO_NONE) return launch_wide_cfg<2, PRO_NONE, false, 4, 2, false, true>(a, g, s);
-            return launch_wide_cfg<2, PRO_GN, false, 4, 2, false, true>(a, g, s);
+            if (a.pro == PRO_NONE) return launch_wide_sel<1, 2, PRO_NONE, false, 4, 2, false, true>(a, g, s);
+            return launch_wide_sel<1, 2, PRO_GN, false, 4, 2, false, true>(a, g, s);
         }
         if (wide_w2(a)) {
-            if (a.pro == PRO_NONE) return launch_wide_cfg<2, PRO_NONE, true, 8, 2, false, true>(a, g, s);
-            return launch_wide_cfg<2, PRO_GN, true, 8, 2, false, true>(a, g, s);
+            if (a.pro == PRO_NONE) return launch_wide_sel<1, 2, PRO_NONE, true, 8, 2, false, true>(a, g, s);
+            return launch_wide_sel<1, 2, PRO_GN, true, 8, 2, false, true>(a, g, s);
         }
         if (a.pro == PRO_NONE) return launch_wide_cfg<2, PRO_NONE, false, 8, 2, false, true>(a, g, s);
         return launch_wide_cfg<2, PRO_GN, false, 8, 2, false, true>(a, g, s);
@@ -1004,14 +1042,14 @@
             if (a.pro == PRO_GN) return launch_wide_cfg<2, PRO_GN, false, 4, 2, false, false, false, true>(a, g, s);
             return launch_wide_cfg<2, PRO_GN_GELU, false, 4, 2, false, false, false, true>(a, g, s);
         }
-        if (a.pro == PRO_NONE) return launch_wide_cfg<2, PRO_NONE, false, 4>(a, g, s);
-        if (a.pro == PRO_GN) return launch_wide_cfg<2, PRO_GN, false, 4>(a, g, s);
-        return launch_wide_cfg<2, PRO_GN_GELU, false, 4>(a, g, s);
+        if (a.pro == PRO_NONE) return launch_wide_sel<1, 2, PRO_NONE, false, 4>(a, g, s);
+        if (a.pro == PRO_GN) return launch_wide_sel<1, 2, PRO_GN, false, 4>(a, g, s);
+        return launch_wide_sel<1, 2, PRO_GN_GELU, false, 4>(a, g, s);
     }
     if (wide_w2(a)) {
-        if (a.pro == PRO_NONE) return launch_wide_cfg<2, PRO_NONE, true>(a, g, s);
-        if (a.pro == PRO_GN) return launch_wide_cfg<2, PRO_GN, true>(a, g, s);
-        return launch_wide_cfg<2, PRO_GN_GELU, true>(a, g, s);
+        if (a.pro == PRO_NONE) return launch_wide_sel<1, 2, PRO_NONE, true>(a, g, s);
+        if (a.pro == PRO_GN) return launch_wide_sel<1, 2, PRO_GN, true>(a, g, s);
+        return launch_wide_sel<1, 2, PRO_GN_GELU, true>(a, g, s);
     }
     if (g.n_tile == 128) {
         if (a.pro == PRO_NONE) return launch_wide_cfg<2, PRO_NONE>(a, g, s);
@@ -1020,18 +1058,18 @@
     }
     if (a.K % 64 == 0 && !(a.sw & SW_WIDE_N64_2X2)) {
         if (pipe) {
-            if (a.pro == PRO_NONE) return launch_wide_cfg<2, PRO_NONE, false, 4, 1, true>(a, g, s);
-            if (a.pro == PRO_GN) return launch_wide_cfg<2, PRO_GN, false, 4, 1, true>(a, g, s);
-            return launch_wide_cfg<2, PRO_GN_GELU, false, 4, 1, true>(a, g, s);
+            if (a.pro == PRO_NONE) return launch_wide_sel<3, 2, PRO_NONE, false, 4, 1, true>(a, g, s);
+            if (a.pro == PRO_GN) return launch_wide_sel<3, 2, PRO_GN, false, 4, 1, true>(a, g, s);
+            return launch_wide_sel<3, 2, PRO_GN_GELU, false, 4, 1, true>(a, g, s);
         }
         if (g2) {
             if (a.pro == PRO_NONE) return launch_wide_cfg<2, PRO_NONE, false, 4, 1, false, false, false, true>(a, g, s);
             if (a.pro == PRO_GN) return launch_wide_cfg<2, PRO_GN, false, 4, 1, false, false, false, true>(a, g, s);
             return launch_wide_cfg<2, PRO_GN_GELU, false, 4, 1, false, false, false, true>(a, g, s);
         }
-        if (a.pro == PRO_NONE) return launch_wide_cfg<2, PRO_NONE, false, 4, 1>(a, g, s);
-        if (a.pro == PRO_GN) return launch_wide_cfg<2, PRO_GN, false, 4, 1>(a, g, s);
-        return launch_wide_cfg<2, PRO_GN_GELU, false, 4, 1>(a, g, s);
+        if (a.pro == PRO_NONE) return launch_wide_sel<3, 2, PRO_NONE, false, 4, 1>(a, g, s);
+        if (a.pro == PRO_GN) return launch_wide_sel<3, 2, PRO_GN, false, 4, 1>(a, g, s);
+        return launch_wide_sel<3, 2, PRO_GN_GELU, false, 4, 1>(a, g, s);
     }
     if (a.pro == PRO_NONE) return launch_wide_cfg<1, PRO_NONE>(a, g, s);
     if (a.pro == PRO_GN) return launch_wide_cfg<1, PRO_GN>(a, g, s);
diff --git a/state_policy_diffusionmodel_amd/csrc/device_utils.h b/state_policy_diffusionmodel_amd/csrc/device_utils.h
--- a/state_policy_diffusionmodel_amd/csrc/device_utils.h
+++ b/state_policy_diffusionmodel_amd/csrc/device_utils.h
@@ -172,15 +172,15 @@
 }
 
 __device__ __forceinline__ float gelu_erf(float v) {
-    const float z = fabsf(v);
-    const float t = __builtin_amdgcn_rcpf(__fmaf_rn(0.3275911f * 0.70710678118654752440f, z, 1.0f));
-    float p = __fmaf_rn(0.5f * 1.061405429f, t, 0.5f * -1.453152027f);
-    p = __fmaf_rn(p, t, 0.5f * 1.421413741f);
-    p = __fmaf_rn(p, t, 0.5f * -0.284496736f);
-    p = __fmaf_rn(p, t, 0.5f * 0.254829592f);
-    const float e = __builtin_amdgcn_exp2f(v * v * -0.72134752044448170368f);
-    const float q = (p * t) * e;
-    return __fmaf_rn(-z, q, fmaxf(v, 0.f));
+    const float x = __builtin_elementwise_minimum(fabsf(v), 6.0f);
+    float e = __fmaf_rn(__builtin_bit_cast(float, 0x3811502cu), x, __builtin_bit_cast(float, 0xba4d288bu));
+    e = __fmaf_rn(e, x, __builtin_bit_cast(float, 0x3c051b28u));
+    e = __fmaf_rn(e, x, __builtin_bit_cast(float, 0xbd5b0c46u));
+    e = __fmaf_rn(e, x, __builtin_bit_cast(float, 0xbeeadd98u));
+    e = __fmaf_rn(e, x, __builtin_bit_cast(float, 0xbf935b1au));
+    e = __fmaf_rn(e, x, __builtin_bit_cast(float, 0xbf7fff70u));
+    const float q = __builtin_amdgcn_exp2f(e);
+    return __fmaf_rn(-x, q, fmaxf(v, 0.f));
 }
 
 __device__ __forceinline__ float wave_sum(float v) {
diff --git a/state_policy_diffusionmodel_amd/csrc/kernels.h b/state_policy_diffusionmodel_amd/csrc/kernels.h
--- a/state_policy_diffusionmodel_amd/csrc/kernels.h
+++ b/state_policy_diffusionmodel_amd/csrc/kernels.h
@@ -40,7 +40,7 @@
     SW_NO_SA_TAIL = 1u << 9, SW_ATTN_VALU = 1u << 10, SW_SA_NO_WLDS = 1u << 11, SW_NO_FILM_FOLD = 1u << 12,
     SW_NO_GRAPH = 1u << 13, SW_NO_SPLITK = 1u << 14, SW_ARENA_TRACE = 1u << 15, SW_NO_WIDE_PIPE = 1u << 16, SW_NO_SKINNY = 1u << 17, SW_DEEP = 1u << 18,
     SW_NO_FILM_LOCAL = 1u << 19, SW_NO_FUSED_SRC = 1u << 20, SW_FILM_LOCAL = 1u << 21, SW_PIN_GEOMETRY = 1u << 22, SW_NO_WP4 = 1u << 23, SW_G2 = 1u << 24, SW_NO_WP8 = 1u << 25, SW_NO_SA_HEAD = 1u << 26, SW_SA_HEAD = 1u << 27, SW_NO_REG64 = 1u << 28,
-    SW_NO_SA_CROP = 1u << 29, SW_NO_SA_OUTC = 1u << 30,
+    SW_NO_SA_CROP = 1u << 29, SW_NO_SA_OUTC = 1u << 30, SW_NO_WHOLE_TILES = 1u << 31,
 };
 struct SwitchName { const char* env; unsigned bit; };
 inline const SwitchName* switch_table(int* n) {
@@ -54,7 +54,7 @@
         {"SPDM_FILM_LOCAL", SW_FILM_LOCAL}, {"SPDM_PIN_GEOMETRY", SW_PIN_GEOMETRY},
         {"SPDM_NO_WP4", SW_NO_WP4}, {"SPDM_G2", SW_G2}, {"SPDM_NO_WP8", SW_NO_WP8},
         {"SPDM_NO_SA_HEAD", SW_NO_SA_HEAD}, {"SPDM_SA_HEAD", SW_SA_HEAD}, {"SPDM_NO_REG64", SW_NO_REG64},
-        {"SPDM_NO_SA_CROP", SW_NO_SA_CROP}, {"SPDM_NO_SA_OUTC", SW_NO_SA_OUTC}};
+        {"SPDM_NO_SA_CROP", SW_NO_SA_CROP}, {"SPDM_NO_SA_OUTC", SW_NO_SA_OUTC}, {"SPDM_NO_WHOLE_TILES", SW_NO_WHOLE_TILES}};
     *n = (int)(sizeof(t) / sizeof(t[0]));
     return t;
 }
@@ -66,7 +66,7 @@
 
 enum { ROUTE_GEMM = 0, ROUTE_SKINNY = 1, ROUTE_REG = 2, ROUTE_WIDE = 3 };
 enum { VAR_PLAIN = 0, VAR_W2 = 1, VAR_WP4 = 2, VAR_WP8 = 3, VAR_PIPE = 4, VAR_G2 = 5 };
-struct GemmRoute { int kernel, variant, m_tile, n_tile; };
+struct GemmRoute { int kernel, variant, m_tile, n_tile, whole; };
 
 struct GemmArgs {
     const float* src;  int src_ld;
diff --git a/state_policy_diffusionmodel_amd/csrc/spdm_api.hip b/state_policy_diffusionmodel_amd/csrc/spdm_api.hip
--- a/state_policy_diffusionmodel_amd/csrc/spdm_api.hip
+++ b/state_policy_diffusionmodel_amd/csrc/spdm_api.hip
@@ -3261,7 +3261,11 @@
     return SPDM_OK;
 }
 
+static int g_op_gemm_whole = -1;
+extern "C" int spdm_debug_whole_tiles(void) { return g_op_gemm_whole; }
+
 extern "C" int spdm_op_gemm(spdm_op_gemm_args* p) {
+    g_op_gemm_whole = -1;
     if (!p) return fail(SPDM_ERR_INVALID, "op_gemm: null argument");
     spdm_op_gemm_args& q = *p;
     for (int i = 0; i < 10; ++i) q.out[i] = -1;
@@ -3336,7 +3340,7 @@
         return fail(SPDM_ERR_INVALID, "op_gemm: this launch does not take a fused source (the plan materialises it)");
     if (two && !gemm_takes_two_sources(a))
         return fail(SPDM_ERR_INVALID, "op_gemm: this launch does not take a two-source input (the plan concatenates)");
-    GemmRoute r{-1, -1, -1, -1};
+    GemmRoute r{-1, -1, -1, -1, 0};
     a.route = &r;
     if (q.epi == EPI_STATS) HIP_TRY(hipMemset(q.d_stats, 0xff, (size_t)q.B * g.slots * 2 * sizeof(double)));
     if (q.d_row_stats) HIP_TRY(hipMemset(q.d_row_stats, 0xff, (size_t)M * g.n_tiles * 2 * sizeof(double)));
@@ -3348,6 +3352,7 @@
                     r.kernel < 0 ? "before any kernel was dispatched (a host-side shape contract)" : "after a kernel was dispatched",
                     hipGetErrorString(es));
     if (es != hipSuccess) return fail(SPDM_ERR_HIP, "op_gemm: %s", hipGetErrorString(es));
+    g_op_gemm_whole = (r.kernel == ROUTE_WIDE) ? r.whole : 0;
     q.out[0] = r.kernel; q.out[1] = r.variant; q.out[2] = r.m_tile; q.out[3] = r.n_tile; q.out[4] = g.ksplit;
     q.out[5] = two ? 1 : 0; q.out[6] = fused ? 1 : 0; q.out[7] = g.slots; q.out[8] = g.st_m_tile; q.out[9] = g.st_n_tiles;
     return SPDM_OK;
```

Measured after the change: 514,000, median of 6. 3.4% higher.
